# awslabs/dgl-ke

Hardware: NVIDIA H100
Metric: edges/sec TransE_l2 d=400 neg=200 at 1/2/4/8 H100 vs ref CPU; HBM GB/s %peak (higher is better)
Workload: dtype f32

## Files before the change

dgl-ke_b200/csrc/kge_abi.cu:

```cuda
#include <cstdio>
#include <unistd.h>
#include <cstdarg>
#include <cstring>
#include <cstdlib>
#include <map>
#include <mutex>
#include <new>
#include <utility>
#include <cuda.h>
#include "kge_common.cuh"

namespace kge {

namespace {
thread_local char g_err[512] = "";
}

int fail(int code, const char* fmt, ...) {
  va_list ap;
  va_start(ap, fmt);
  vsnprintf(g_err, sizeof(g_err), fmt, ap);
  va_end(ap);
  return code;
}

int smem_optin(const void* kernel, size_t bytes) {
  if (bytes <= 48 * 1024) return KGE_OK;
  if (bytes > kSmemOptinMax) return fail(KGE_ERR_UNSUPPORTED, "%zu bytes of shared memory per CTA requested, sm_90 allows %zu", bytes, kSmemOptinMax);
  int dev = 0;
  cudaGetDevice(&dev);
  static std::mutex mu;
  static std::map<std::pair<const void*, int>, size_t> done;
  std::lock_guard<std::mutex> lock(mu);
  size_t& have = done[{kernel, dev}];
  if (bytes <= have) return KGE_OK;
  const cudaError_t e = cudaFuncSetAttribute(kernel, cudaFuncAttributeMaxDynamicSharedMemorySize, (int)bytes);
  if (e != cudaSuccess) {
    cudaGetLastError();
    return fail(KGE_ERR_CUDA, "cudaFuncSetAttribute(MaxDynamicSharedMemorySize, %zu): %s", bytes, cudaGetErrorString(e));
  }
  have = bytes;
  return KGE_OK;
}

struct Buffer {
  void* p = nullptr;
  size_t bytes = 0;
  bool host = false;
  template <class T> T* as() const { return static_cast<T*>(p); }

  void release() {
    if (p) host ? cudaFreeHost(p) : cudaFree(p);
    p = nullptr;
    bytes = 0;
  }
  int resize(size_t n, cudaStream_t stream, const char* what) {
    cudaStreamCaptureStatus cs = cudaStreamCaptureStatusNone;
    cudaStreamIsCapturing(stream, &cs);
    if (cs != cudaStreamCaptureStatusNone)
      return fail(KGE_ERR_INVALID_ARG, "the %s must be (re)allocated (%zu bytes, has %zu) but the stream is capturing: "
                  "run one eager step first", what, n, bytes);
    cudaError_t e = cudaStreamSynchronize(stream);
    if (e != cudaSuccess) return fail(KGE_ERR_CUDA, "cudaStreamSynchronize before reallocating the %s: %s", what, cudaGetErrorString(e));
    release();
    e = host ? cudaMallocHost(&p, n) : cudaMalloc(&p, n);
    if (e != cudaSuccess) {
      p = nullptr;
      cudaGetLastError();
      return fail(KGE_ERR_NOMEM, "%s(%zu) for the %s failed: %s", host ? "cudaMallocHost" : "cudaMalloc", n, what,
                  cudaGetErrorString(e));
    }
    bytes = n;
    return KGE_OK;
  }
};

}
using namespace kge;

#define KGE_CUDA_OK(expr)                                                                      \
  do {                                                                                         \
    cudaError_t e_ = (expr);                                                                   \
    if (e_ != cudaSuccess) return fail(KGE_ERR_CUDA, "%s: %s", #expr, cudaGetErrorString(e_)); \
  } while (0)

struct kge_context {
  int device = 0;
  int num_sms = 0;
  long long launches = 0;
  int engine = -1;
  int rel_deferred = 0;
  Buffer arena;
  float* ng_ptr = nullptr;
  size_t ng_floats = 0;
  bool ng_dirty = false;
  Buffer pin{nullptr, 0, true};
  Buffer dev_stage;
  float* red_partial = nullptr;
  Buffer rel_dense;
  float* ext_rg = nullptr;
  float* ext_rgs = nullptr;
  float* dump_v = nullptr;
  Buffer negdeg_ids;
  struct Prefetch {
    bool armed = false;
    kge_batch_t next{};
    long long next_nneg = 0;
    bool ready = false;
    const void *r_nodes = nullptr, *r_negs = nullptr, *r_nU_dev = nullptr;
    long long r_nU = 0, r_nneg = 0;
    int r_buf = 0;
    Buffer nc[2];
    Buffer bn[2];
    FusedPrefetch args{};

    void take_staged(const kge_batch_t& b, bool usable, StepParams& p, StepWs& w) {
      if (!ready) return;
      ready = false;
      if (usable && r_nodes == b.node_ids && r_negs == b.neg_ids && r_nU == b.n_nodes &&
          r_nU_dev == (b.n_nodes < 0 ? b.n_nodes_dev : nullptr) && r_nneg == p.Nn) {
        w.NC = nc[r_buf].as<float>();
        w.BnRaw = bn[r_buf].as<float>();
        p.nc_staged = 1;
      }
    }

    int arm_next(bool usable, StepParams& p, StepWs& w, float* arena_nc, cudaStream_t stream, const FusedPrefetch** out) {
      *out = nullptr;
      if (!armed) return KGE_OK;
      armed = false;
      const long long ncap = 2 * p.B;
      const long long nU = next.n_nodes < 0 ? ncap : next.n_nodes;
      if (!usable || nU > ncap || next_nneg <= 0 || fused_prefetch_slots(p, 0) < 2 || fused_prefetch_slots(p, 1) < 2)
        return KGE_OK;
      const size_t ncb = (size_t)ncap * p.D * sizeof(float), bnb = (size_t)next_nneg * p.D * sizeof(float);
      if (ncb > nc[0].bytes || ncb > nc[1].bytes || bnb > bn[0].bytes || bnb > bn[1].bytes) {
        for (int i = 0; i < 2; ++i) {
          int rc;
          if ((rc = nc[i].resize(ncb, stream, "prefetch staging buffers")) || (rc = bn[i].resize(bnb, stream, "prefetch staging buffers")))
            return rc;
        }
        w.BnRaw = nullptr; w.NC = arena_nc; p.nc_staged = 0;
      }
      const int tgt = p.nc_staged ? (r_buf ^ 1) : 0;
      const void* nU_dev = next.n_nodes < 0 ? next.n_nodes_dev : nullptr;
      args = FusedPrefetch{(const long long*)next.node_ids, (const long long*)nU_dev, nU, (const long long*)next.neg_ids,
                           next_nneg, nc[tgt].as<float>(), bn[tgt].as<float>()};
      ready = true;
      r_nodes = next.node_ids; r_negs = next.neg_ids; r_nU = next.n_nodes; r_nU_dev = nU_dev; r_nneg = next_nneg; r_buf = tgt;
      *out = &args;
      return KGE_OK;
    }
  } pf;
  int fused_mode = -1;
  float* dev_log4 = nullptr;
  StepParams last_p{};
  StepWs last_w{};
  BatchView last_b{};
  TableView last_ent{}, last_rel{};
  bool have_last = false;
  Profiler prof;
};

namespace {

struct DeviceGuard {
  int prev = -1;
  explicit DeviceGuard(int dev) {
    cudaGetDevice(&prev);
    if (prev != dev) cudaSetDevice(dev);
    else prev = -1;
  }
  ~DeviceGuard() {
    if (prev >= 0) cudaSetDevice(prev);
  }
};

int make_view(const kge_table_t* t, TableView* v, const char* what) {
  if (!t || !t->shards) return fail(KGE_ERR_INVALID_ARG, "%s table is null", what);
  if (t->n_shards < 1 || t->n_shards > KGE_MAX_SHARDS)
    return fail(KGE_ERR_INVALID_ARG, "%s table: n_shards=%d out of [1,%d]", what, t->n_shards, KGE_MAX_SHARDS);
  if (t->dim <= 0 || t->num_rows <= 0) return fail(KGE_ERR_INVALID_ARG, "%s table: empty", what);
  memset(v, 0, sizeof(*v));
  v->n_shards = t->n_shards;
  v->dim = t->dim;
  v->num_rows = t->num_rows;
  v->rows_per_shard = (t->num_rows + t->n_shards - 1) / t->n_shards;
  for (int s = 0; s < t->n_shards; ++s) {
    const kge_shard_t& sh = t->shards[s];
    long long begin = (long long)s * v->rows_per_shard;
    long long end = begin + v->rows_per_shard;
    if (end > t->num_rows) end = t->num_rows;
    if (sh.row_begin != begin || sh.row_end != end || sh.dim != t->dim)
      return fail(KGE_ERR_INVALID_ARG, "%s table: shard %d must cover rows [%lld,%lld) with dim %d", what, s, begin,
                  end, t->dim);
    if (!sh.emb || !sh.state_sum) return fail(KGE_ERR_INVALID_ARG, "%s table: shard %d has null pointers", what, s);
    if (((uintptr_t)sh.emb & 15) != 0) return fail(KGE_ERR_INVALID_ARG, "%s table: shard %d not 16-byte aligned", what, s);
    v->emb[s] = sh.emb;
    v->state[s] = sh.state_sum;
  }
  return KGE_OK;
}

int make_params(const kge_step_cfg_t* cfg, long long n_nodes, StepParams* p) {
  if (!cfg) return fail(KGE_ERR_INVALID_ARG, "cfg is null");
  if (cfg->model < KGE_TRANSE_L1 || cfg->model > KGE_ROTATE) return fail(KGE_ERR_INVALID_ARG, "unknown model %d", cfg->model);
  if (cfg->batch <= 0 || cfg->chunk_size <= 0 || cfg->neg_sample_size <= 0)
    return fail(KGE_ERR_INVALID_ARG, "batch/chunk_size/neg_sample_size must be positive");
  if (cfg->batch % cfg->chunk_size != 0)
    return fail(KGE_ERR_INVALID_ARG, "batch %lld is not a multiple of chunk_size %d", (long long)cfg->batch, cfg->chunk_size);
  const int D = cfg->entity_dim, Dr = cfg->relation_dim;
  if (D <= 0 || Dr <= 0) return fail(KGE_ERR_INVALID_ARG, "dims must be positive");
  if (D % 4 != 0 || Dr % 4 != 0)
    return fail(KGE_ERR_UNSUPPORTED, "row lengths must be multiples of 4 floats (16-byte vector/TMA access): D_e=%d D_r=%d", D, Dr);
  switch (cfg->model) {
    case KGE_TRANSE_L1: case KGE_TRANSE_L2: case KGE_DISTMULT:
      if (Dr != D) return fail(KGE_ERR_INVALID_ARG, "model needs relation_dim == entity_dim (%d vs %d)", Dr, D);
      break;
    case KGE_COMPLEX:
      if (Dr != D || D % 8 != 0) return fail(KGE_ERR_INVALID_ARG, "ComplEx needs relation_dim == entity_dim, a multiple of 8");
      break;
    case KGE_ROTATE:
      if (D != 2 * Dr || D % 8 != 0) return fail(KGE_ERR_INVALID_ARG, "RotatE needs entity_dim == 2*relation_dim (-de), a multiple of 8");
      break;
    case KGE_RESCAL:
      if (Dr != D * D) return fail(KGE_ERR_INVALID_ARG, "RESCAL needs relation_dim == entity_dim^2");
      if (D > 512) return fail(KGE_ERR_UNSUPPORTED, "RESCAL entity_dim %d > 512 is not implemented", D);
      break;
  }
  p->model = cfg->model; p->D = D; p->Dr = Dr;
  p->gamma = cfg->gamma; p->emb_init = cfg->emb_init; p->lr = cfg->lr;
  p->reg_coef = cfg->reg_coef; p->reg_norm = cfg->reg_norm;
  p->adversarial = cfg->adversarial; p->adv_temperature = cfg->adv_temperature;
  p->neg_head = cfg->neg_head ? 1 : 0;
  p->B = cfg->batch; p->Cs = cfg->chunk_size; p->Ns = cfg->neg_sample_size;
  p->C = (int)(cfg->batch / cfg->chunk_size);
  p->neg_deg = cfg->neg_deg_sample ? 1 : 0;
  if (p->neg_deg) p->Ns += p->Cs;
  p->Nn = (long long)p->C * p->Ns;
  p->U = n_nodes >= 0 ? n_nodes : 2 * p->B;
  p->U_dev = nullptr;
  p->rel_deferred = 0; p->rel_dense = 0; p->use_nc = 1; p->fused = 0; p->nc_staged = 0;
  if (cfg->loss_genre < KGE_LOSS_LOGSIGMOID || cfg->loss_genre > KGE_LOSS_BCE)
    return fail(KGE_ERR_INVALID_ARG, "loss_genre %d is not a kge_loss_t", cfg->loss_genre);
  if (cfg->pairwise && cfg->loss_genre != KGE_LOSS_HINGE && cfg->loss_genre != KGE_LOSS_LOGISTIC)
    return fail(KGE_ERR_INVALID_ARG, "pairwise needs the Hinge or the Logistic criterion (loss.py:61-62)");
  if (cfg->pairwise && cfg->adversarial)
    return fail(KGE_ERR_INVALID_ARG, "loss cannot be pairwise and adversarial sampled (base_loss.py:83-84)");
  p->hinge = cfg->loss_genre == KGE_LOSS_HINGE ? 1 : 0;
  p->margin = cfg->margin;
  p->pairwise = cfg->pairwise ? 1 : 0;
  return KGE_OK;
}

size_t align_up(size_t x, size_t a = 256) { return (x + a - 1) / a * a; }

struct CarveOpt {
  bool force_tiles = false;
  bool want_scores = true;
};

bool use_fused(kge_context* h, const StepParams& p) {
  return h->engine != 0 && h->fused_mode != 0 && fused_supported(p);
}

bool use_umma(kge_context* h, const StepParams& p) {
  return h->engine != 0 && umma_supported(p);
}

int carve(kge_context* h, const StepParams& p, StepWs* w, cudaStream_t stream, const CarveOpt& opt = CarveOpt()) {
  const size_t BD = (size_t)p.B * p.D, ND = (size_t)p.Nn * p.D, BNs = (size_t)p.B * p.Ns;
  const size_t B = (size_t)p.B, Nn = (size_t)p.Nn, U = (size_t)(p.U > 0 ? p.U : 0);
  const bool um = !opt.force_tiles && use_umma(h, p);
  const bool fused = p.fused != 0;
  const size_t sA = B * slab_blocks(p.D) * 32 + 8192, sB = Nn * slab_blocks(p.D) * 32 + 8192;
  const size_t sV = B * slab_blocks(p.Ns) * 32 + 8192;
  const size_t sAT = (size_t)p.C * slab_blocks(p.Cs) * p.D * 32 + 8192, sBT = (size_t)p.C * slab_blocks(p.Ns) * p.D * 32 + 8192;
  const size_t sVT = (size_t)p.C * slab_blocks(p.Cs) * p.Ns * 32 + 8192;
  struct Slot { float** ptr; size_t floats; bool on; };
  const Slot slots[] = {
      {&w->NG, (U ? 2 * B : 0) * p.D, true},
      {&w->A, BD, !(um || fused)}, {&w->Bn, ND, true}, {&w->GA, BD, true}, {&w->GR, B * p.Dr, !p.rel_dense},
      {&w->S, BNs, !fused || opt.want_scores}, {&w->V, BNs, !fused},
      {&w->pos, B, true}, {&w->gpos, B, true}, {&w->pnorm, B, true}, {&w->a2, B, true}, {&w->b2, Nn, true},
      {&w->rowsum, B, true}, {&w->colsum, Nn, true}, {&w->pl, B, true}, {&w->nl, B, true}, {&w->wbar, 4, true},
      {&w->gsr, B, true}, {&w->gsn, Nn, true}, {&w->colpart, (size_t)ceil_div(p.Cs, 128) * Nn, fused},
      {&w->Mt, BD, p.model == KGE_RESCAL},
      {&w->Ahi, sA, um}, {&w->Alo, sA, um}, {&w->Bhi, sB, um}, {&w->Blo, sB, um},
      {&w->Vhi, sV, um && !fused}, {&w->Vlo, sV, um && !fused},
      {&w->AhiT, sAT, um}, {&w->AloT, sAT, um}, {&w->BhiT, sBT, um}, {&w->BloT, sBT, um},
      {&w->VhiT, sVT, um}, {&w->VloT, sVT, um},
      {&w->NC, U * p.D, p.use_nc != 0},
      {&w->regp, B + Nn + (U ? 2 * B : 0), true},
  };
  size_t need = 0;
  for (const Slot& s : slots)
    if (s.on) need += align_up(s.floats * sizeof(float));
  if (need > h->arena.bytes) {
    if (int rc = h->arena.resize(need + need / 4, stream, "step workspace")) return rc;
    h->ng_ptr = nullptr; h->ng_floats = 0;
  }
  size_t off = 0;
  for (const Slot& s : slots) {
    *s.ptr = s.on ? (float*)(h->arena.as<char>() + off) : nullptr;
    if (s.on) off += align_up(s.floats * sizeof(float));
  }
  w->red_partial = h->red_partial; w->red_ticket = (unsigned int*)(h->red_partial + 192);
  w->sync_ctr = (unsigned int*)(h->red_partial + 200);
  w->rg = nullptr; w->rgs = nullptr;
  return KGE_OK;
}

int ensure_rel_dense(kge_context* h, const TableView& rel, StepWs* w, cudaStream_t stream) {
  const size_t bytes = ((size_t)rel.num_rows * rel.dim + (size_t)rel.num_rows) * sizeof(float);
  if (bytes != h->rel_dense.bytes) {
    if (int rc = h->rel_dense.resize(bytes, stream, "relation gradient sums")) return rc;
    KGE_CUDA_OK(cudaMemsetAsync(h->rel_dense.p, 0, bytes, stream));
  }
  w->rg = h->rel_dense.as<float>();
  w->rgs = w->rg + (size_t)rel.num_rows * rel.dim;
  return KGE_OK;
}

LaunchCtx lctx(kge_context* h, void* stream) { return LaunchCtx{(cudaStream_t)stream, &h->launches, h->num_sms, &h->prof}; }

void ensure_ng_zero(kge_context* h, const StepParams& p, const StepWs& w, const LaunchCtx& c, bool force) {
  size_t n = (size_t)2 * p.B * p.D;
  if (force || h->ng_dirty || h->ng_ptr != w.NG || h->ng_floats < n) {
    launch_fill_zero(c, w.NG, (long long)n);
    h->ng_ptr = w.NG;
    h->ng_dirty = false;
  }
  h->ng_floats = n;
}

int check_batch(const kge_batch_t* b, const StepParams& p) {
  if (!b) return fail(KGE_ERR_INVALID_ARG, "batch is null");
  if (!b->node_ids || !b->head_local || !b->tail_local || !b->rel_ids || !b->neg_ids)
    return fail(KGE_ERR_INVALID_ARG, "batch has null index arrays");
  if (b->n_nodes < 0 && b->n_nodes_dev) return KGE_OK;
  if (b->n_nodes <= 0 || b->n_nodes > 2 * p.B) return fail(KGE_ERR_INVALID_ARG, "n_nodes=%lld out of (0, 2*batch]", (long long)b->n_nodes);
  return KGE_OK;
}

BatchView bview(const kge_batch_t* b) {
  return BatchView{(const long long*)b->node_ids, (const long long*)b->head_local, (const long long*)b->tail_local,
                   (const long long*)b->rel_ids, (const long long*)b->neg_ids, b->edge_weight,
                   (const long long*)b->head_ids, (const long long*)b->tail_ids};
}

int run_score(kge_context* h, const LaunchCtx& c, const StepParams& p, const StepWs& w) {
  if (use_umma(h, p)) return umma_score(c, p, w);
  launch_score(c, p, w);
  return KGE_OK;
}

}

extern "C" {

KGE_API int kge_abi_version(void) { return KGE_ABI_VERSION; }
KGE_API const char* kge_last_error(void) { return g_err; }

KGE_API int kge_create(int device, kge_handle_t* out) {
  if (!out) return fail(KGE_ERR_INVALID_ARG, "out is null");
  *out = nullptr;
  int n = 0;
  cudaError_t e = cudaGetDeviceCount(&n);
  if (e != cudaSuccess || n == 0) {
    cudaGetLastError();
    return fail(KGE_ERR_NO_DEVICE, "no CUDA device visible (%s); libkge_b200 has no CPU path", cudaGetErrorString(e));
  }
  if (device < 0 || device >= n) return fail(KGE_ERR_INVALID_ARG, "device %d out of range [0,%d)", device, n);
  cudaDeviceProp prop;
  KGE_CUDA_OK(cudaGetDeviceProperties(&prop, device));
  if (prop.major != 9)
    return fail(KGE_ERR_NO_DEVICE, "device %d is sm_%d%d; this library is built for sm_90a (H100) only", device, prop.major, prop.minor);
  kge_context* h = new (std::nothrow) kge_context();
  if (!h) return fail(KGE_ERR_NOMEM, "out of host memory");
  h->device = device;
  h->num_sms = prop.multiProcessorCount;
  if (const char* ev = getenv("KGE_B200_FUSED")) h->fused_mode = atoi(ev) ? 1 : 0;

  DeviceGuard g(device);
  if (cudaMalloc(&h->dev_log4, 4 * sizeof(float)) != cudaSuccess) { delete h; return fail(KGE_ERR_NOMEM, "cudaMalloc failed"); }

  if (cudaMalloc(&h->red_partial, 256 * sizeof(float)) != cudaSuccess || cudaMemset(h->red_partial, 0, 256 * sizeof(float)) != cudaSuccess) {
    delete h; return fail(KGE_ERR_NOMEM, "cudaMalloc failed");
  }
  *out = h;
  return KGE_OK;
}

KGE_API int kge_destroy(kge_handle_t h) {
  if (!h) return KGE_OK;
  DeviceGuard g(h->device);
  cudaDeviceSynchronize();
  for (Buffer* b : {&h->arena, &h->dev_stage, &h->pin, &h->rel_dense, &h->negdeg_ids, &h->pf.nc[0], &h->pf.nc[1],
                    &h->pf.bn[0], &h->pf.bn[1]})
    b->release();
  if (h->dev_log4) cudaFree(h->dev_log4);
  if (h->red_partial) cudaFree(h->red_partial);
  if (h->prof.created)
    for (int i = 0; i < Profiler::kMax; ++i) { cudaEventDestroy(h->prof.ev0[i]); cudaEventDestroy(h->prof.ev1[i]); }
  delete h;
  return KGE_OK;
}

KGE_API int64_t kge_launch_count(kge_handle_t h) { return h ? h->launches : 0; }

KGE_API int kge_profile_enable(kge_handle_t h, int on) {
  if (!h) return fail(KGE_ERR_INVALID_ARG, "handle is null");
  DeviceGuard g(h->device);
  Profiler& p = h->prof;
  if (on && !p.created) {
    for (int i = 0; i < Profiler::kMax; ++i) {
      KGE_CUDA_OK(cudaEventCreate(&p.ev0[i]));
      KGE_CUDA_OK(cudaEventCreate(&p.ev1[i]));
    }
    p.created = true;
  }
  p.enabled = on != 0;
  p.n = 0;
  return KGE_OK;
}

KGE_API int kge_profile_read(kge_handle_t h, char* names, int names_len, float* ms, int max_records) {
  if (!h || !names || !ms) return fail(KGE_ERR_INVALID_ARG, "null argument");
  DeviceGuard g(h->device);
  Profiler& p = h->prof;
  KGE_CUDA_OK(cudaDeviceSynchronize());
  int n = p.n < max_records ? p.n : max_records, off = 0;
  names[0] = 0;
  for (int i = 0; i < n; ++i) {
    KGE_CUDA_OK(cudaEventElapsedTime(&ms[i], p.ev0[i], p.ev1[i]));
    int w = snprintf(names + off, names_len - off, "%s%s", i ? "|" : "", p.names[i]);
    if (w < 0 || off + w >= names_len) break;
    off += w;
  }
  p.n = 0;
  return n;
}

KGE_API int kge_set_engine(kge_handle_t h, int engine) {
  if (!h) return fail(KGE_ERR_INVALID_ARG, "handle is null");
  if (engine < -1 || engine > 1) return fail(KGE_ERR_INVALID_ARG, "engine must be -1, 0 or 1");
  h->engine = engine;
  return KGE_OK;
}

KGE_API int kge_set_fused(kge_handle_t h, int mode) {
  if (!h) return fail(KGE_ERR_INVALID_ARG, "handle is null");
  if (mode < -1 || mode > 1) return fail(KGE_ERR_INVALID_ARG, "mode must be -1, 0 or 1");
  h->fused_mode = mode;
  return KGE_OK;
}

KGE_API int kge_debug_set_dump(kge_handle_t h, float* coef_dump) {
  if (!h) return fail(KGE_ERR_INVALID_ARG, "handle is null");
  h->dump_v = coef_dump;
  return KGE_OK;
}

KGE_API int kge_gather(kge_handle_t h, const kge_table_t* table, const int64_t* idx, int64_t n, float* out, void* stream) {
  if (!h) return fail(KGE_ERR_INVALID_ARG, "handle is null");
  if (n < 0) return fail(KGE_ERR_INVALID_ARG, "n < 0");
  if (n == 0) return KGE_OK;
  if (!idx || !out) return fail(KGE_ERR_INVALID_ARG, "idx/out is null");
  TableView v;
  int rc = make_view(table, &v, "gather");
  if (rc) return rc;
  DeviceGuard g(h->device);
  launch_gather(lctx(h, stream), v, (const long long*)idx, n, out);
  KGE_CUDA_OK(cudaGetLastError());
  return KGE_OK;
}

KGE_API int kge_score_pos(kge_handle_t h, const kge_step_cfg_t* cfg, const float* head, const float* rel, const float* tail,
                  int64_t n, float* out, void* stream) {
  if (!h) return fail(KGE_ERR_INVALID_ARG, "handle is null");
  if (!cfg) return fail(KGE_ERR_INVALID_ARG, "cfg is null");
  if (n == 0) return KGE_OK;
  if (!head || !rel || !tail || !out || n < 0) return fail(KGE_ERR_INVALID_ARG, "bad arguments");
  kge_step_cfg_t c2 = *cfg;
  c2.batch = n; c2.chunk_size = (int32_t)1; c2.neg_sample_size = 1;
  if (n > 0x7fffffffLL) return fail(KGE_ERR_INVALID_ARG, "n too large");
  StepParams p;
  int rc = make_params(&c2, 0, &p);
  if (rc) return rc;
  DeviceGuard g(h->device);
  StepWs w{};
  w.pos = out;
  LaunchCtx c = lctx(h, stream);
  if (p.model == KGE_RESCAL) launch_rescal_prep_dense(c, p, head, rel, tail, w, true, false);
  else launch_prep_dense(c, p, head, rel, tail, nullptr, w, true, false);
  KGE_CUDA_OK(cudaGetLastError());
  return KGE_OK;
}

KGE_API int kge_score_neg(kge_handle_t h, const kge_step_cfg_t* cfg, const float* heads, const float* rel, const float* tails,
                  float* out, void* stream) {
  if (!h) return fail(KGE_ERR_INVALID_ARG, "handle is null");
  if (!heads || !rel || !tails || !out) return fail(KGE_ERR_INVALID_ARG, "null pointer");
  StepParams p;
  int rc = make_params(cfg, 0, &p);
  if (rc) return rc;
  DeviceGuard g(h->device);
  StepWs w{};
  CarveOpt opt;
  opt.force_tiles = (p.model == KGE_RESCAL);
  rc = carve(h, p, &w, (cudaStream_t)stream, opt);
  if (rc) return rc;
  h->ng_ptr = nullptr;
  LaunchCtx c = lctx(h, stream);
  const float* negrows = p.neg_head ? heads : tails;
  if (p.model == KGE_RESCAL) launch_rescal_prep_dense(c, p, heads, rel, tails, w, false, true);
  else launch_prep_dense(c, p, heads, rel, tails, negrows, w, false, true);
  StepWs w2 = w;
  w2.Bn = const_cast<float*>(negrows);
  w2.S = out;
  if (opt.force_tiles) launch_score(c, p, w2);
  else rc = run_score(h, c, p, w2);
  if (rc) return rc;
  KGE_CUDA_OK(cudaGetLastError());
  h->have_last = false;
  return KGE_OK;
}

KGE_API int kge_loss_grad(kge_handle_t h, const kge_step_cfg_t* cfg, const float* pos, const float* neg, const float* wt,
                  float* dpos, float* dneg, float* log4, void* stream) {
  if (!h) return fail(KGE_ERR_INVALID_ARG, "handle is null");
  if (!pos || !neg || !dpos || !dneg) return fail(KGE_ERR_INVALID_ARG, "null pointer");
  StepParams p;
  int rc = make_params(cfg, 0, &p);
  if (rc) return rc;
  p.model = KGE_DISTMULT;
  DeviceGuard g(h->device);
  StepWs w{};
  rc = carve(h, p, &w, (cudaStream_t)stream);
  if (rc) return rc;
  h->ng_ptr = nullptr;
  w.V = dneg;
  w.gpos = dpos;
  launch_loss(lctx(h, stream), p, pos, neg, wt, w, log4, false);
  KGE_CUDA_OK(cudaGetLastError());
  h->have_last = false;
  return KGE_OK;
}

KGE_API int kge_adagrad(kge_handle_t h, const kge_table_t* table, const int64_t* idx, const float* grad, int64_t n, float lr,
                void* stream) {
  if (!h) return fail(KGE_ERR_INVALID_ARG, "handle is null");
  if (n < 0) return fail(KGE_ERR_INVALID_ARG, "n < 0");
  if (n == 0) return KGE_OK;
  if (!idx || !grad) return fail(KGE_ERR_INVALID_ARG, "null pointer");
  TableView v;
  int rc = make_view(table, &v, "adagrad");
  if (rc) return rc;
  DeviceGuard g(h->device);
  launch_adagrad(lctx(h, stream), v, (const long long*)idx, grad, n, lr);
  KGE_CUDA_OK(cudaGetLastError());
  return KGE_OK;
}

static int forward_backward_impl(kge_handle_t h, const kge_step_cfg_t* cfg, const kge_table_t* ent, const kge_table_t* rel,
                                 const kge_batch_t* batch, float* log4, void* stream, bool fused_step) {
  if (!h) return fail(KGE_ERR_INVALID_ARG, "handle is null");
  StepParams p;
  int rc = make_params(cfg, batch ? batch->n_nodes : 0, &p);
  if (rc) return rc;
  rc = check_batch(batch, p);
  if (rc) return rc;
  if (batch->n_nodes < 0) p.U_dev = (const long long*)batch->n_nodes_dev;
  p.rel_deferred = h->rel_deferred;
  TableView ve, vr;
  if ((rc = make_view(ent, &ve, "entity"))) return rc;
  if ((rc = make_view(rel, &vr, "relation"))) return rc;
  if (ve.dim != p.D || vr.dim != p.Dr)
    return fail(KGE_ERR_INVALID_ARG, "table dims (%d,%d) do not match cfg (%d,%d)", ve.dim, vr.dim, p.D, p.Dr);
  DeviceGuard g(h->device);
  p.fused = use_fused(h, p) ? 1 : 0;
  p.use_nc = (fused_step && ve.n_shards == 1) ? 0 : 1;
  p.rel_dense = (fused_step && p.model != KGE_RESCAL &&
                 (p.rel_deferred ? (h->ext_rg != nullptr) : ((size_t)vr.num_rows * (size_t)vr.dim <= ((size_t)64 << 20)))) ? 1 : 0;
  StepWs w{};
  CarveOpt opt;
  opt.want_scores = !fused_step;
  if ((rc = carve(h, p, &w, (cudaStream_t)stream, opt))) return rc;
  if (p.rel_dense && p.rel_deferred) { w.rg = h->ext_rg; w.rgs = h->ext_rgs; }
  else if (p.rel_dense && (rc = ensure_rel_dense(h, vr, &w, (cudaStream_t)stream))) return rc;
  LaunchCtx c = lctx(h, stream);
  BatchView b = bview(batch);
  if (p.neg_deg) {
    if (ve.n_shards != 1) return fail(KGE_ERR_UNSUPPORTED, "--neg_deg_sample needs a single-shard entity table");
// ... 478 lines not shown
```

dgl-ke_b200/csrc/kge_common.cuh:

```cuda
#pragma once
#include <cuda_runtime.h>
#include <stdint.h>
#include "../../include/kge_b200.h"

namespace kge {

constexpr int kWarp = 32;

struct TableView {
  float* emb[KGE_MAX_SHARDS];
  float* state[KGE_MAX_SHARDS];
  long long rows_per_shard;
  long long num_rows;
  int n_shards;
  int dim;
};

__device__ __forceinline__ float* row_ptr(const TableView& t, long long id) {
  if (t.n_shards == 1) return t.emb[0] + id * (long long)t.dim;
  int s = (int)(id / t.rows_per_shard);
  return t.emb[s] + (id - (long long)s * t.rows_per_shard) * (long long)t.dim;
}
__device__ __forceinline__ float* state_ptr(const TableView& t, long long id) {
  if (t.n_shards == 1) return t.state[0] + id;
  int s = (int)(id / t.rows_per_shard);
  return t.state[s] + (id - (long long)s * t.rows_per_shard);
}

struct StepParams {
  int model;
  int D;
  int Dr;
  float gamma, emb_init, lr, reg_coef;
  int reg_norm;
  int adversarial;
  float adv_temperature;
  int neg_head;
  long long B;
  int C, Cs, Ns;
  long long Nn;
  long long U;
  const long long* U_dev;
  int rel_deferred;
  int rel_dense;
  int use_nc;
  int fused;
  int hinge;
  float margin;
  int pairwise;
  int neg_deg;
  int nc_staged;
};

__host__ __device__ __forceinline__ bool node_reg_in_update(const StepParams& p) { return !p.use_nc || p.nc_staged; }

struct StepWs {
  float* A;
  float* Bn;
  float* GA;
  float* GR;
  float* NG;
  float* NC;
  float* S;
  float* V;
  float* pos;
  float* gpos;
  float* pnorm;
  float* a2;
  float* b2;
  float* rowsum;
  float* colsum;
  float* pl;
  float* nl;
  float* regp;
  float* wbar;
  float* gsr;
  float* gsn;
  float* colpart;
  float* rg;
  float* rgs;
  const float* BnRaw;
  unsigned int* sync_ctr;
  float* red_partial;
  unsigned int* red_ticket;
  float* Mt;
  float *Ahi, *Alo;
  float *Bhi, *Blo;
  float *Vhi, *Vlo;
  float *AhiT, *AloT;
  float *BhiT, *BloT;
  float *VhiT, *VloT;
};

struct BatchView {
  const long long* node_ids;
  const long long* head_local;
  const long long* tail_local;
  const long long* rel_ids;
  const long long* neg_ids;
  const float* edge_weight;
  const long long* head_ids;
  const long long* tail_ids;
};

__device__ __forceinline__ long long node_count(const StepParams& p) { return p.U_dev ? *p.U_dev : p.U; }

__device__ __forceinline__ const float* node_row(const StepParams& p, const TableView& ent, const BatchView& b,
                                                 const StepWs& w, long long loc) {
  return p.use_nc ? (w.NC + loc * (long long)p.D) : row_ptr(ent, b.node_ids[loc]);
}
__device__ __forceinline__ const float* head_row(const StepParams& p, const TableView& ent, const BatchView& b,
                                                 const StepWs& w, long long i) {
  if (!p.use_nc && b.head_ids) return row_ptr(ent, b.head_ids[i]);
  return node_row(p, ent, b, w, b.head_local[i]);
}
__device__ __forceinline__ const float* tail_row(const StepParams& p, const TableView& ent, const BatchView& b,
                                                 const StepWs& w, long long i) {
  if (!p.use_nc && b.tail_ids) return row_ptr(ent, b.tail_ids[i]);
  return node_row(p, ent, b, w, b.tail_local[i]);
}

__device__ __forceinline__ float warp_sum(float v) {
#pragma unroll
  for (int o = 16; o > 0; o >>= 1) v += __shfl_xor_sync(0xffffffffu, v, o);
  return v;
}
__device__ __forceinline__ float warp_max(float v) {
#pragma unroll
  for (int o = 16; o > 0; o >>= 1) v = fmaxf(v, __shfl_xor_sync(0xffffffffu, v, o));
  return v;
}

__device__ __forceinline__ float4 ld4(const float* p) { return *reinterpret_cast<const float4*>(p); }
__device__ __forceinline__ void st4(float* p, float4 v) { *reinterpret_cast<float4*>(p) = v; }
__device__ __forceinline__ float4 ld4_stream(const float* p) {
  float4 r;
  asm volatile("ld.global.L1::no_allocate.v4.f32 {%0,%1,%2,%3}, [%4];"
               : "=f"(r.x), "=f"(r.y), "=f"(r.z), "=f"(r.w) : "l"(p));
  return r;
}
__device__ __forceinline__ void red_add4(float* p, float4 v) {
  asm volatile("red.global.add.v4.f32 [%0], {%1,%2,%3,%4};"
               :: "l"(p), "f"(v.x), "f"(v.y), "f"(v.z), "f"(v.w) : "memory");
}

__device__ __forceinline__ void red_add4_sys(float* p, float4 v) {
  asm volatile("red.relaxed.sys.global.add.v4.f32 [%0], {%1,%2,%3,%4};"
               :: "l"(p), "f"(v.x), "f"(v.y), "f"(v.z), "f"(v.w) : "memory");
}
__device__ __forceinline__ void table_red_add4(const TableView& t, float* p, float4 v) {
  if (t.n_shards > 1) red_add4_sys(p, v); else red_add4(p, v);
}
__device__ __forceinline__ void table_atomic_add(const TableView& t, float* p, float v) {
  if (t.n_shards > 1) atomicAdd_system(p, v); else atomicAdd(p, v);
}

#define KGE_F4_OP2(name, expr)                                                     \
  __device__ __forceinline__ float4 name(float4 a, float4 b) {                     \
    float4 r;                                                                      \
    { float x = a.x, y = b.x; r.x = (expr); } { float x = a.y, y = b.y; r.y = (expr); } \
    { float x = a.z, y = b.z; r.z = (expr); } { float x = a.w, y = b.w; r.w = (expr); } \
    return r;                                                                      \
  }
KGE_F4_OP2(f4_add, x + y)
KGE_F4_OP2(f4_sub, x - y)
KGE_F4_OP2(f4_mul, x* y)
#undef KGE_F4_OP2
__device__ __forceinline__ float4 f4_scale(float4 a, float s) { return make_float4(a.x * s, a.y * s, a.z * s, a.w * s); }
__device__ __forceinline__ float4 f4_neg(float4 a) { return make_float4(-a.x, -a.y, -a.z, -a.w); }
__device__ __forceinline__ float4 f4_fma(float4 a, float s, float4 c) {
  return make_float4(fmaf(a.x, s, c.x), fmaf(a.y, s, c.y), fmaf(a.z, s, c.z), fmaf(a.w, s, c.w));
}
__device__ __forceinline__ float f4_hsum(float4 a) { return (a.x + a.y) + (a.z + a.w); }
__device__ __forceinline__ float f4_dot(float4 a, float4 b) { return f4_hsum(f4_mul(a, b)); }
__device__ __forceinline__ float sgnf(float x) { return (x > 0.f) ? 1.f : ((x < 0.f) ? -1.f : 0.f); }

__device__ __forceinline__ void split_tf32(float x, float& hi, float& lo) {
  uint32_t hb, lb;
  asm("cvt.rna.tf32.f32 %0, %1;" : "=r"(hb) : "f"(x));
  hi = __uint_as_float(hb);
  asm("cvt.rna.tf32.f32 %0, %1;" : "=r"(lb) : "f"(x - hi));
  lo = __uint_as_float(lb);
}
__device__ __forceinline__ void split_tf32_4(float4 v, float4& h, float4& l) {
  split_tf32(v.x, h.x, l.x); split_tf32(v.y, h.y, l.y); split_tf32(v.z, h.z, l.z); split_tf32(v.w, h.w, l.w);
}
__host__ __device__ inline int slab_blocks(int ncol) { return (ncol + 31) >> 5; }
__device__ __forceinline__ long long slab_off(long long chunk, int nblk, int R, int row, int col) {
  return ((chunk * nblk + (col >> 5)) * (long long)R + row) * 32 + (col & 31);
}
__device__ __forceinline__ long long slabT_off(long long chunk, int R, int Ncol, int row, int col) {
  return ((chunk * slab_blocks(R) + (row >> 5)) * (long long)Ncol + col) * 32 + (row & 31);
}
constexpr int kPrepRows = 32;
constexpr size_t kSmemOptinMax = 227 * 1024;
__host__ __device__ inline int prep_stage_stride(int D) { return ((D + 27) & ~31) + 4; }
inline size_t prep_stage_bytes(int D) { return (size_t)kPrepRows * prep_stage_stride(D) * sizeof(float); }
inline bool prep_stage_fits(int D) { return prep_stage_bytes(D) <= kSmemOptinMax; }

struct RowOut {
  float* f32;
  float* hi;
  float* lo;
  long long chunk;
  int nblk, R, row;
  float* stage;
};
__device__ __forceinline__ void row_store4(const RowOut& o, int col, float4 v) {
  if (o.f32) *reinterpret_cast<float4*>(o.f32 + col) = v;
  if (o.hi) {
    float4 h, l;
    split_tf32_4(v, h, l);
    const long long off = slab_off(o.chunk, o.nblk, o.R, o.row, col);
    *reinterpret_cast<float4*>(o.hi + off) = h;
    *reinterpret_cast<float4*>(o.lo + off) = l;
  }
  if (o.stage) *reinterpret_cast<float4*>(o.stage + col) = v;
}

static __device__ __noinline__ float abs_pow_generic(float ax, int p) { return powf(ax, (float)p); }
__device__ __forceinline__ float abs_pow(float x, int p) {
  float ax = fabsf(x);
  if (p == 3) return ax * ax * ax;
  if (p == 2) return ax * ax;
  if (p == 1) return ax;
  return abs_pow_generic(ax, p);
}
static __device__ __noinline__ float reg_grad_pow(float x, int p, float coef) {
  return coef * (float)p * powf(fabsf(x), (float)(p - 1)) * sgnf(x);
}
__device__ __forceinline__ float reg_grad(float x, int p, float coef) {
  if (coef == 0.f || p <= 0) return 0.f;
  float ax = fabsf(x);
  if (p == 3) return 3.f * coef * ax * x;
  if (p == 2) return 2.f * coef * x;
  if (p == 1) return coef * sgnf(x);
  return reg_grad_pow(x, p, coef);
}
__device__ __forceinline__ float4 reg_grad4(float4 x, int p, float coef) {
  return make_float4(reg_grad(x.x, p, coef), reg_grad(x.y, p, coef), reg_grad(x.z, p, coef), reg_grad(x.w, p, coef));
}
__device__ __forceinline__ float abs_pow4_sum(float4 x, int p) {
  return (abs_pow(x.x, p) + abs_pow(x.y, p)) + (abs_pow(x.z, p) + abs_pow(x.w, p));
}

__device__ __forceinline__ float softplusf(float s) { return fmaxf(s, 0.f) + log1pf(expf(-fabsf(s))); }
__device__ __forceinline__ float sigmoidf(float s) {
  if (s >= 0.f) return 1.f / (1.f + expf(-s));
  float e = expf(s);
  return e / (1.f + e);
}

inline int ceil_div(long long a, long long b) { return (int)((a + b - 1) / b); }

int fail(int code, const char* fmt, ...);
int smem_optin(const void* kernel, size_t bytes);

struct Profiler {
  static constexpr int kMax = 64;
  bool enabled = false;
  int n = 0;
  const char* names[kMax];
  cudaEvent_t ev0[kMax], ev1[kMax];
  bool created = false;
};

struct LaunchCtx {
  cudaStream_t stream;
  long long* launch_counter;
  int num_sms;
  Profiler* prof;
};

inline void prof_begin(const LaunchCtx& c, const char* name) {
  Profiler* p = c.prof;
  if (!p || !p->enabled || p->n >= Profiler::kMax) return;
  p->names[p->n] = name;
  cudaEventRecord(p->ev0[p->n], c.stream);
}
inline void prof_end(const LaunchCtx& c) {
  Profiler* p = c.prof;
  if (!p || !p->enabled || p->n >= Profiler::kMax) return;
  cudaEventRecord(p->ev1[p->n], c.stream);
  ++p->n;
}

#define KGE_LAUNCH_NAMED(ctx, name, kernel, grid, block, smem, ...)            \
  do {                                                                          \
    prof_begin((ctx), name);                                                    \
    kernel<<<(grid), (block), (smem), (ctx).stream>>>(__VA_ARGS__);             \
    prof_end((ctx));                                                            \
    if ((ctx).launch_counter) ++*(ctx).launch_counter;                          \
  } while (0)

#define KGE_LAUNCH(ctx, kernel, grid, block, smem, ...)                         \
  do {                                                                          \
    prof_begin((ctx), #kernel);                                                 \
    kernel<<<(grid), (block), (smem), (ctx).stream>>>(__VA_ARGS__);             \
    prof_end((ctx));                                                            \
    if ((ctx).launch_counter) ++*(ctx).launch_counter;                          \
  } while (0)

struct SamplerParams {
  const long long *heads, *rels, *tails;
  long long n_edges, n_entities;
  long long B, Nn;
  unsigned long long seed;
  int half_bits;
  long long *o_head, *o_rel, *o_tail;
  long long *o_neg;
  long long *o_nodes, *o_hl, *o_tl;
  long long* o_n_nodes;
  unsigned long long* tkey;
  int* tpos;
  int* tloc;
  int hmask;
  int* flags;
};

void launch_sampler(const LaunchCtx&, const SamplerParams&, long long step);

void launch_gather(const LaunchCtx&, const TableView& t, const long long* idx, long long n, float* out);
void launch_gather_nodes(const LaunchCtx&, const StepParams&, const TableView& ent, const BatchView&, const StepWs&);
int launch_prep(const LaunchCtx&, const StepParams&, const TableView& ent, const TableView& rel,
                const BatchView&, const StepWs&);
int launch_prep_nonedge(const LaunchCtx&, const StepParams&, const TableView& ent, const TableView& rel,
                        const BatchView&, const StepWs&);
void launch_prep_dense(const LaunchCtx&, const StepParams&, const float* head, const float* relr,
                       const float* tail, const float* negrows, const StepWs&, bool want_pos, bool want_a);
void launch_score(const LaunchCtx&, const StepParams&, const StepWs&);
void launch_loss(const LaunchCtx&, const StepParams&, const float* pos, const float* S, const float* w,
                 const StepWs&, float* log4, bool want_reg);
void launch_wbar(const LaunchCtx&, const StepParams&, const float* w, const StepWs&);
void launch_loss_rows(const LaunchCtx&, const StepParams&, const float* pos, const float* S, const float* w, const StepWs&);
void launch_colsum(const LaunchCtx&, const StepParams&, const StepWs&);
void launch_reduce_log(const LaunchCtx&, const StepParams&, const float* w, const StepWs&, float* log4, bool want_reg);
void launch_grad_a(const LaunchCtx&, const StepParams&, const StepWs&);
void launch_grad_b(const LaunchCtx&, const StepParams&, const StepWs&);
void launch_chain(const LaunchCtx&, const StepParams&, const TableView& ent, const TableView& rel,
                  const BatchView&, const StepWs&);
int launch_update(const LaunchCtx&, const StepParams&, const TableView& ent, const TableView& rel,
                  const BatchView&, const StepWs&, float* log4, const float* wt);
void launch_adagrad(const LaunchCtx&, const TableView& t, const long long* idx, const float* grad,
                    long long n, float lr);
void launch_node_grad_with_reg(const LaunchCtx&, const StepParams&, const TableView& ent,
                               const BatchView&, const StepWs&, float* out);
void launch_fill_zero(const LaunchCtx&, float* p, long long n);
void launch_rel_grad_dense(const LaunchCtx&, const StepParams&, const BatchView&, const StepWs&, float* rg, float* rgs);
void launch_rel_apply_dense(const LaunchCtx&, const TableView& rel, float* rg, float* rgs, float lr);

void launch_negdeg_ids(const LaunchCtx&, const StepParams&, const BatchView&, const long long* sampled, long long* out);
void launch_negdeg_zero_reg(const LaunchCtx&, const StepParams&, const StepWs&);
void launch_negdeg_mask_scores(const LaunchCtx&, const StepParams&, const StepWs&);
void launch_negdeg_mask_coef(const LaunchCtx&, const StepParams&, const StepWs&);
void launch_negdeg_scatter(const LaunchCtx&, const StepParams&, const TableView& ent, const BatchView&, const StepWs&);

int launch_rescal_prep(const LaunchCtx&, const StepParams&, const TableView& ent, const TableView& rel,
                       const BatchView&, const StepWs&);
void launch_rescal_prep_dense(const LaunchCtx&, const StepParams&, const float* head, const float* relr,
                              const float* tail, const StepWs&, bool want_pos, bool want_a);
void launch_rescal_chain(const LaunchCtx&, const StepParams&, const TableView& ent, const TableView& rel,
                         const BatchView&, const StepWs&);

bool umma_supported(const StepParams&);
int umma_score(const LaunchCtx&, const StepParams&, const StepWs&);
int umma_grad(const LaunchCtx&, const StepParams&, const StepWs&, bool side_b);

struct FusedPrefetch {
  const long long* node_ids;
  const long long* nU_dev;
  long long nU;
  const long long* neg_ids;
  long long nNeg;
  float* nc;
  float* bn;
};
bool fused_supported(const StepParams&);
int fused_prefetch_slots(const StepParams& p, int mode);
int fused_launch(const LaunchCtx&, const StepParams&, const StepWs&, int mode, const float* wt, float* dumpS, float* dumpV,
                 const TableView* ent, const long long* neg_ids, const FusedPrefetch* pf);

}
```

dgl-ke_b200/csrc/kge_fused.cu:

```cuda
#include <cuda.h>
#include <cstdio>
#include <cstdlib>
#include <mutex>
#include "kge_common.cuh"
#include "kge_tc.cuh"

namespace kge {

using namespace tc;

namespace {

constexpr int kTileM = 128;
constexpr int kThreadsF = 384;
constexpr int kProducerWarp = 8;
constexpr int kHandoffWarp = 9;
constexpr int kMaxS1 = 4, kMaxS2 = 8;
constexpr int kMaxPf = 8;
constexpr uint32_t kRingBytes = 192 * 1024;
constexpr uint32_t kRingBytesP = 223 * 1024;
constexpr float kLog2e = 1.4426950408889634f;
constexpr float kLn2 = 0.6931471805599453f;

struct FusedArgs {
  int model, adversarial;
  float gamma, Tl2e, inv2B, uni;
  float reg_coef;
  int reg_norm;
  int C, Rx, Ry, D;
  int N1;
  int N2;
  int nblkD;
  int nS1, nS2;
  uint32_t stage1Bytes, stage2Bytes;
  float *VhiT, *VloT;
  float* colpart;
  int ncolpart;
  const float* x2;
  const float* y2;
  const float* pos;
  const float* wt;
  const float* wbar;
  float *gpos, *rowsum, *pl, *nl;
  float* dumpS;
  float* dumpV;
  const float *Xhi, *Xlo;
  const long long* xids;
  TableView xtab;
  const float* xraw;
  float* gsn;
  float* out;
  int pf_slots;
  int pf_parity;
  int pf_lag;
  uint32_t pf_off, pf_row_bytes;
  const long long* pf_node_ids;
  const long long* pf_nU_dev;
  long long pf_nU, pf_nNeg;
  const long long* pf_neg_ids;
  float* pf_nc;
  float* pf_bn;
};

static __device__ __noinline__ float reg_grad_any(float b, int norm, float coef) { return reg_grad(b, norm, coef); }
__device__ __forceinline__ float reg_grad_fast(float b, int norm, float coef) {
  if (norm == 3) return 3.f * coef * fabsf(b) * b;
  return reg_grad_any(b, norm, coef);
}

__device__ __forceinline__ void epi_bar() { asm volatile("bar.sync 1, 256;" ::: "memory"); }

__device__ __forceinline__ void prefetch_rows(const FusedArgs& g, uint8_t* ring, uint64_t (*pf_full)[kMaxPf], int w, int lane) {
  const int S = g.pf_slots;
  const long long nU = g.pf_nU_dev ? *g.pf_nU_dev : g.pf_nU;
  const long long total = nU + g.pf_nNeg;
  const long long nhalf = total > g.pf_parity ? (total - g.pf_parity + 1) / 2 : 0;
  const long long stride = 2ll * gridDim.x, j0 = 2ll * blockIdx.x + w;
  const long long n = j0 < nhalf ? (nhalf - j0 + stride - 1) / stride : 0;
  uint8_t* slots = ring + g.pf_off + (size_t)w * S * g.pf_row_bytes;
  auto vrow = [&](long long k) { return g.pf_parity + 2 * (j0 + k * stride); };
  auto fetch_ids = [&](long long kb) {
    const long long k = kb + lane;
    if (k >= n) return 0ll;
    const long long v = vrow(k);
    return v < nU ? g.pf_node_ids[v] : g.pf_neg_ids[v - nU];
  };
  long long ids_lo = fetch_ids(0), ids_hi = fetch_ids(32);
  long long base = 0;
  auto load = [&](long long k) {
    const int o = (int)(k - base);
    const long long id = __shfl_sync(0xffffffffu, o < 32 ? ids_lo : ids_hi, o & 31);
    const int s = (int)(k % S);
    if (elect_one()) {
      mbar_expect_tx(&pf_full[w][s], g.pf_row_bytes);
      bulk_g2s(slots + (size_t)s * g.pf_row_bytes, row_ptr(g.xtab, id), g.pf_row_bytes, &pf_full[w][s]);
    }
    __syncwarp();
  };
  for (long long k = 0; k < n && k < S; ++k) load(k);
  const int L = g.pf_lag < S - 1 ? g.pf_lag : (S > 2 ? S - 2 : 1);
  for (long long k = 0; k < n; ++k) {
    const int s = (int)(k % S);
    mbar_wait(&pf_full[w][s], (uint32_t)((k / S) & 1));
    const long long v = vrow(k);
    float* dst = v < nU ? g.pf_nc + v * (long long)g.D : g.pf_bn + (v - nU) * (long long)g.D;
    const long long kr = k - L + S;
    const bool reload = k >= L && kr < n;
    if (reload && kr >= base + 32) { base += 32; ids_lo = ids_hi; ids_hi = fetch_ids(base + 32); }
    if (elect_one()) {
      bulk_s2g(dst, slots + (size_t)s * g.pf_row_bytes, g.pf_row_bytes);
      bulk_commit();
      if (reload) { if (L == 3) bulk_wait_read<3>(); else if (L == 2) bulk_wait_read<2>(); else bulk_wait_read<1>(); }
    }
    __syncwarp();
    if (reload) load(kr);
  }
  if (elect_one()) bulk_wait_all();
  __syncwarp();
}

template <int NW, int KS>
__device__ __forceinline__ void kblock_3xtf32(float (&acc)[NW / 2], uint64_t dXh, uint64_t dXl, uint64_t dYh, uint64_t dYl) {
  wgmma_fence();
#pragma unroll
  for (int ks = 0; ks < KS; ++ks) {
    const uint64_t o = (uint64_t)(ks * 2);
    wgmma_ss<NW>(acc, dXh + o, dYh + o, 1u);
    wgmma_ss<NW>(acc, dXh + o, dYl + o, 1u);
    wgmma_ss<NW>(acc, dXl + o, dYh + o, 1u);
  }
  wgmma_commit();
}

template <int NV>
__device__ __forceinline__ int vsm_idx(int i, int k) {
  const int g = i & 7, h = (i >> 3) & 1, kk = k & 7;
  const int L = 4 * g + (kk & 3);
  return (((i >> 4) * (NV / 8) + (k >> 3)) * 32 + (L ^ ((L >> 3) & 3))) * 4 + h + 2 * (kk >> 2);
}

template <int NW>
__device__ __forceinline__ void pos_kstep(float (&acc2)[NW / 2], uint32_t (&ah)[4], uint32_t (&al)[4], const float* vf,
                                          uint64_t dYh, uint64_t dYl) {
  const float4 v = *reinterpret_cast<const float4*>(vf);
  const float a[4] = {v.x, v.y, v.z, v.w};
#pragma unroll
  for (int r = 0; r < 4; ++r) {
    float hi, lo;
    split_tf32(a[r], hi, lo);
    ah[r] = __float_as_uint(hi); al[r] = __float_as_uint(lo);
  }
  wgmma_fence();
  wgmma_rs<NW>(acc2, ah, dYh, 1u);
  wgmma_rs<NW>(acc2, ah, dYl, 1u);
  wgmma_rs<NW>(acc2, al, dYh, 1u);
  wgmma_commit();
}

__device__ __forceinline__ int tile_row() {
  uint32_t t;
  asm volatile("mov.u32 %0, %%tid.x;" : "=r"(t));
  return (int)((t >> 5) * 16 + ((t >> 2) & 7));
}

template <int NV, int NW>
__global__ void __launch_bounds__(kThreadsF, 1)
k_fused_pos(const __grid_constant__ CUtensorMap mXh, const __grid_constant__ CUtensorMap mXl,
            const __grid_constant__ CUtensorMap mYh1, const __grid_constant__ CUtensorMap mYl1,
            const __grid_constant__ CUtensorMap mYh2, const __grid_constant__ CUtensorMap mYl2, FusedArgs g) {
  extern __shared__ __align__(1024) uint8_t smem_raw[];
  __shared__ __align__(8) uint64_t full1[kMaxS1], empty1[kMaxS1], full2[kMaxS2], empty2[kMaxS2];
  __shared__ __align__(8) uint64_t vfree;
  __shared__ __align__(8) uint64_t pf_full[2][kMaxPf];
  __shared__ __align__(16) float colA[NV];
  __shared__ float rsc[kTileM];

  const int warp = threadIdx.x >> 5, lane = threadIdx.x & 31;
  uint8_t* ring = (uint8_t*)(((uintptr_t)smem_raw + 1023) & ~(uintptr_t)1023);
  float* vsm = reinterpret_cast<float*>(ring);
  constexpr uint32_t vBytes = (uint32_t)NV * 512u;
  uint8_t* ring2 = ring + vBytes;

  const int mtiles = (g.Rx + kTileM - 1) / kTileM;
  const int ntiles = g.C * mtiles;
  const int nkb1 = (g.D + 31) >> 5;
  const int nkb2 = (g.Ry + 31) >> 5;
  const int nchunks = (g.D + NW - 1) / NW;
  constexpr uint32_t yBytes1 = (uint32_t)NV * 128u;
  constexpr uint32_t yBytes2 = (uint32_t)NW * 128u;
  const bool l2 = g.model == KGE_TRANSE_L2;
  const int nhand = g.pf_slots > 0 ? 1 : 3;
  const uint32_t hand_bar_n = 256u + 32u * (uint32_t)nhand;

  if (threadIdx.x == 0) {
    for (int s = 0; s < kMaxS1; ++s) { mbar_init(&full1[s], 1); mbar_init(&empty1[s], 8); }
    for (int s = 0; s < kMaxS2; ++s) { mbar_init(&full2[s], 1); mbar_init(&empty2[s], 8); }
    mbar_init(&vfree, 8 + nhand);
    for (int s = 0; s < kMaxPf; ++s) { mbar_init(&pf_full[0][s], 1); mbar_init(&pf_full[1][s], 1); }
    asm volatile("fence.mbarrier_init.release.cluster;" ::: "memory");
  }
  if (warp == kProducerWarp && lane == 0) {
    tma_prefetch_desc(&mXh); tma_prefetch_desc(&mXl); tma_prefetch_desc(&mYh1);
    tma_prefetch_desc(&mYl1); tma_prefetch_desc(&mYh2); tma_prefetch_desc(&mYl2);
  }
  __syncthreads();

  if (warp >= 8) {
  asm volatile("setmaxnreg.dec.sync.aligned.u32 56;");
  if (warp == kProducerWarp) {
    uint32_t n1 = 0, n2 = 0, it = 0;
    for (int tile = blockIdx.x; tile < ntiles; tile += gridDim.x, ++it) {
      const int c = tile / mtiles, m0 = (tile % mtiles) * kTileM;
      if (it > 0) mbar_wait(&vfree, (it - 1) & 1);
      for (int kb = 0; kb < nkb1; ++kb, ++n1) {
        const uint32_t s = n1 % g.nS1;
        mbar_wait(&empty1[s], ((n1 / g.nS1) & 1) ^ 1);
        uint8_t* st = ring + (size_t)s * g.stage1Bytes;
        const int yx = (c * g.nblkD + kb) * g.Rx + m0;
        const int yy = (c * g.nblkD + kb) * g.Ry;
        if (elect_one()) {
          mbar_expect_tx(&full1[s], 2u * 16384u + 2u * yBytes1);
          tma_load_2d(st, &mXh, &full1[s], 0, yx);
          tma_load_2d(st + 16384, &mXl, &full1[s], 0, yx);
          tma_load_2d(st + 32768, &mYh1, &full1[s], 0, yy);
          tma_load_2d(st + 32768 + yBytes1, &mYl1, &full1[s], 0, yy);
        }
        __syncwarp();
      }
      for (uint32_t k = (n1 > (uint32_t)g.nS1 ? n1 - g.nS1 : 0); k < n1; ++k) mbar_wait(&empty1[k % g.nS1], (k / g.nS1) & 1);
      for (int ch = 0; ch < nchunks; ++ch) {
        for (int kb = 0; kb < nkb2; ++kb, ++n2) {
          const uint32_t s = n2 % g.nS2;
          mbar_wait(&empty2[s], ((n2 / g.nS2) & 1) ^ 1);
          uint8_t* st = ring2 + (size_t)s * g.stage2Bytes;
          const int yy = (c * nkb2 + kb) * g.D + ch * NW;
          if (elect_one()) {
            mbar_expect_tx(&full2[s], 2u * yBytes2);
            tma_load_2d(st, &mYh2, &full2[s], 0, yy);
            tma_load_2d(st + yBytes2, &mYl2, &full2[s], 0, yy);
          }
          __syncwarp();
        }
      }
    }
  } else if (warp - kHandoffWarp < nhand) {
    const int hw = warp - kHandoffWarp;
    for (int tile = blockIdx.x; tile < ntiles; tile += gridDim.x) {
      const int c = tile / mtiles, m0 = (tile % mtiles) * kTileM;
      const int rows = g.Rx - m0 < kTileM ? g.Rx - m0 : kTileM;
      const int nb = (rows + 31) >> 5;
      asm volatile("bar.sync 2, %0;" ::"r"(hand_bar_n) : "memory");
      float* dst = g.colpart + (long long)(tile % mtiles) * g.C * g.Ry + (long long)c * g.Ry;
      for (int j = hw; j < g.Ry; j += nhand) {
        float s = 0.f;
        float v[kTileM / 32];
#pragma unroll
        for (int b = 0; b < kTileM / 32; ++b) {
          const int i = 32 * b + lane;
          v[b] = b < nb ? vsm[vsm_idx<NV>(i, j)] * rsc[i] : 0.f;
        }
#pragma unroll
        for (int b = 0; b < kTileM / 32; ++b) {
          const int i = 32 * b + lane;
          if (i < rows) {
            float hi, lo;
            split_tf32(v[b], hi, lo);
            const long long o = slabT_off(c, g.Rx, g.Ry, m0 + i, j);
            g.VhiT[o] = hi; g.VloT[o] = lo;
          }
          s += v[b];
        }
        if (l2) {
#pragma unroll
          for (int x = 16; x >= 1; x >>= 1) s += __shfl_xor_sync(0xffffffffu, s, x);
          if (lane == 0) dst[j] = s;
        }
      }
      asm volatile("fence.proxy.async.shared::cta;" ::: "memory");
      __syncwarp();
      if (lane == 0) mbar_arrive(&vfree);
    }
  } else if (warp >= 10 && g.pf_slots > 0) {
    prefetch_rows(g, ring, pf_full, warp - 10, lane);
  }
  } else {
    asm volatile("setmaxnreg.inc.sync.aligned.u32 224;");
    const int wg = warp >> 2, q = lane & 3;
    const int et = threadIdx.x;
    uint32_t n1 = 0, n2 = 0;
    for (int tile = blockIdx.x; tile < ntiles; tile += gridDim.x) {
      const int c = tile / mtiles, m0 = (tile % mtiles) * kTileM;
      epi_bar();
      for (int y = et; y < NV; y += 256) {
        const bool ok = y < g.Ry;
        colA[y] = (l2 && ok) ? g.y2[(long long)c * g.Ry + y] : 0.f;
      }
      epi_bar();
      float rscal[2];
      {
      float acc[NV / 2];
#pragma unroll
      for (int i = 0; i < NV / 2; ++i) acc[i] = 0.f;
      for (int kb = 0; kb < nkb1; ++kb, ++n1) {
        const uint32_t s = n1 % g.nS1;
        mbar_wait(&full1[s], (n1 / g.nS1) & 1);
        const uint32_t st = smem_u32(ring + (size_t)s * g.stage1Bytes);
        const uint64_t dXh = make_desc(st + wg * 8192u), dXl = make_desc(st + 16384u + wg * 8192u);
        const uint64_t dYh = make_desc(st + 32768u), dYl = make_desc(st + 32768u + yBytes1);
        const int kleft = g.D - kb * 32;
        const int ksteps = kleft >= 32 ? 4 : (kleft >> 3);
        switch (ksteps) {
          case 4: kblock_3xtf32<NV, 4>(acc, dXh, dXl, dYh, dYl); break;
          case 3: kblock_3xtf32<NV, 3>(acc, dXh, dXl, dYh, dYl); break;
          case 2: kblock_3xtf32<NV, 2>(acc, dXh, dXl, dYh, dYl); break;
          default: kblock_3xtf32<NV, 1>(acc, dXh, dXl, dYh, dYl); break;
        }
        if (kb > 0) {
          wgmma_wait<1>();
          if (lane == 0) mbar_arrive(&empty1[(n1 - 1) % g.nS1]);
        }
      }
      wgmma_wait<0>();
      if (lane == 0) mbar_arrive(&empty1[(n1 - 1) % g.nS1]);
      reg_fence(acc);
      epi_bar();
      const int rloc = tile_row();

#pragma unroll
      for (int h = 0; h < 2; ++h) {
        const int m = m0 + rloc + 8 * h;
        const bool row_ok = m < g.Rx;
        const long long gx = (long long)c * g.Rx + (row_ok ? m : 0);
        const float x2v = (l2 && row_ok) ? g.x2[gx] : 0.f;
        const float w_i = (g.wt && row_ok) ? g.wt[gx] : 1.f;
        const float kw = w_i * g.inv2B;
        float mxl = -INFINITY;
        if (g.adversarial || g.dumpS) {
#pragma unroll
          for (int j = 0; j < NV / 8; ++j) {
            float sv[2];
#pragma unroll
            for (int e = 0; e < 2; ++e) {
              const int col = 8 * j + 2 * q + e;
              float s = acc[4 * j + 2 * h + e];
              if (l2) {
                const float sqc = fmaxf(fmaf(-2.f, s, colA[col]) + x2v, 1e-30f);
                s = g.gamma - sqc * rsqrta(sqc);
              }
              sv[e] = s;
              if (col < g.Ry) mxl = fmaxf(mxl, s * g.Tl2e);
            }
            if (g.dumpS && row_ok && 8 * j + 2 * q < g.Ry)
              *reinterpret_cast<float2*>(g.dumpS + gx * g.Ry + 8 * j + 2 * q) = make_float2(sv[0], sv[1]);
          }
        }
        if (g.adversarial) {
          mxl = fmaxf(mxl, __shfl_xor_sync(0xffffffffu, mxl, 1));
          mxl = fmaxf(mxl, __shfl_xor_sync(0xffffffffu, mxl, 2));
        } else {
          mxl = 0.f;
        }
        float nls = 0.f, rs = 0.f, den = 0.f;
#pragma unroll
        for (int j = 0; j < NV / 8; ++j) {
#pragma unroll
          for (int e = 0; e < 2; ++e) {
            const int col = 8 * j + 2 * q + e;
            float s = acc[4 * j + 2 * h + e], rinv = 1.f;
            if (l2) {
              const float sq = fmaf(-2.f, s, colA[col]) + x2v;
              const float sqc = fmaxf(sq, 1e-30f);
              const float r = rsqrta(sqc);
              s = g.gamma - sqc * r;
              rinv = (sq > 1e-30f) ? r : 0.f;
            }
            const float pe = g.adversarial ? ex2a(fmaf(s, g.Tl2e, -mxl)) : 1.f;
            const float t = ex2a(-fabsf(s) * kLog2e);
            const float u = 1.f + t;
            const float r1 = rcpa(u);
            const float sig = (s >= 0.f) ? r1 : t * r1;
            const float sp = fmaf(kLn2, lg2a(u), fmaxf(s, 0.f));
            const bool ok = row_ok && (col < g.Ry);
            const float coef = ok ? pe * sig * kw * rinv : 0.f;
            if (ok) { nls = fmaf(pe, sp, nls); den += pe; }
            rs += coef;
            vsm[vsm_idx<NV>(rloc + 8 * h, col)] = coef;
          }
        }
        den += __shfl_xor_sync(0xffffffffu, den, 1); den += __shfl_xor_sync(0xffffffffu, den, 2);
        nls += __shfl_xor_sync(0xffffffffu, nls, 1); nls += __shfl_xor_sync(0xffffffffu, nls, 2);
        rs += __shfl_xor_sync(0xffffffffu, rs, 1); rs += __shfl_xor_sync(0xffffffffu, rs, 2);
        const float rscale = g.adversarial ? (row_ok ? 1.f / den : 0.f) : g.uni;
        rscal[h] = rscale;
        if (g.dumpV && row_ok) {
          for (int j = 0; j < NV / 8; ++j)
            if (8 * j + 2 * q < g.Ry)
              *reinterpret_cast<float2*>(g.dumpV + gx * g.Ry + 8 * j + 2 * q) =
                  make_float2(vsm[vsm_idx<NV>(rloc + 8 * h, 8 * j + 2 * q)] * rscale,
                              vsm[vsm_idx<NV>(rloc + 8 * h, 8 * j + 2 * q + 1)] * rscale);
        }
        if (q == 0 && row_ok) {
          const float ps = g.pos[gx];
          const float wb = g.wt ? *g.wbar : 1.f;
          g.pl[gx] = softplusf(-ps);
          g.nl[gx] = nls * rscale * w_i;
          g.gpos[gx] = -sigmoidf(-ps) * wb * g.inv2B;
          if (l2) g.rowsum[gx] = rs * rscale;
        }
      }
      if (q == 0) { rsc[rloc] = rscal[0]; rsc[rloc + 8] = rscal[1]; }
      }
      asm volatile("bar.arrive 2, %0;" ::"r"(hand_bar_n) : "memory");
      __syncwarp();

      const float* vw = vsm + ((warp * (NV / 8)) * 32 + (lane ^ ((lane >> 3) & 3))) * 4;
      const int rloc = tile_row();
      for (int ch = 0; ch < nchunks; ++ch) {
        const int d0 = ch * NW;
        float acc2[NW / 2];
#pragma unroll
        for (int i = 0; i < NW / 2; ++i) acc2[i] = 0.f;
        uint32_t ah[2][4], al[2][4];
#pragma unroll 1
        for (int kb = 0; kb < nkb2; ++kb) {
          const uint32_t s = n2 % g.nS2;
          mbar_wait(&full2[s], (n2 / g.nS2) & 1);
          const uint32_t st = smem_u32(ring2 + (size_t)s * g.stage2Bytes);
          const uint64_t dYh = make_desc(st), dYl = make_desc(st + yBytes2);
          const int kleft = g.Ry - kb * 32;
          const int ksteps = kleft >= 32 ? 4 : (kleft >> 3);
#pragma unroll
          for (int ks = 0; ks < 4; ++ks) {
            const int j = kb * 4 + ks;
            if (ks < ksteps) {
              const uint64_t o = (uint64_t)(ks * 2);
              pos_kstep<NW>(acc2, ah[j & 1], al[j & 1], vw + j * 128, dYh + o, dYl + o);
              if (j > 0) {
                wgmma_wait<1>();
                reg_fence(ah[(j - 1) & 1]); reg_fence(al[(j - 1) & 1]);
                if (ks == 0 && lane == 0) mbar_arrive(&empty2[(n2 - 1) % g.nS2]);
              }
            }
          }
          ++n2;
        }
        wgmma_wait<0>();
        reg_fence(ah[0]); reg_fence(ah[1]); reg_fence(al[0]); reg_fence(al[1]);
        if (lane == 0) mbar_arrive(&empty2[(n2 - 1) % g.nS2]);
        reg_fence(acc2);
#pragma unroll
        for (int h = 0; h < 2; ++h) {
          const int m = m0 + rloc + 8 * h;
          if (m >= g.Rx) continue;
          float* orow = g.out + ((long long)c * g.Rx + m) * (long long)g.D;
#pragma unroll
          for (int j = 0; j < NW / 8; ++j) {
            const int k = d0 + 8 * j + 2 * q;
            if (k >= g.D) continue;
            *reinterpret_cast<float2*>(orow + k) = make_float2(acc2[4 * j + 2 * h] * rscal[h], acc2[4 * j + 2 * h + 1] * rscal[h]);
          }
        }
      }
      asm volatile("fence.proxy.async.shared::cta;" ::: "memory");
      __syncwarp();
      if (lane == 0) mbar_arrive(&vfree);
    }
  }
}

constexpr int kNegEpiLoads = 16;

template <int NW, bool FLAT>
__global__ void __launch_bounds__(kThreadsF, 1)
k_fused_neg(const __grid_constant__ CUtensorMap mVh, const __grid_constant__ CUtensorMap mVl,
            const __grid_constant__ CUtensorMap mAh, const __grid_constant__ CUtensorMap mAl, FusedArgs g) {
  extern __shared__ __align__(1024) uint8_t smem_raw[];
  __shared__ __align__(8) uint64_t full[kMaxS1], empty[kMaxS1];
  __shared__ __align__(8) uint64_t pf_full[2][kMaxPf];

  const int warp = threadIdx.x >> 5, lane = threadIdx.x & 31;
  uint8_t* ring = (uint8_t*)(((uintptr_t)smem_raw + 1023) & ~(uintptr_t)1023);

  const int mtiles = (g.Rx + kTileM - 1) / kTileM;
  const int ntiles = g.C * mtiles;
  const int nkb = (g.Ry + 31) >> 5;
  const int nch = (g.D + NW - 1) / NW;
  constexpr uint32_t aBytes = (uint32_t)kTileM * 128u;
  constexpr uint32_t bBytes = (uint32_t)NW * 128u;
  const bool l2 = g.model == KGE_TRANSE_L2;

  if (threadIdx.x == 0) {
    for (int s = 0; s < kMaxS1; ++s) { mbar_init(&full[s], 1); mbar_init(&empty[s], 8); }
    for (int s = 0; s < kMaxPf; ++s) { mbar_init(&pf_full[0][s], 1); mbar_init(&pf_full[1][s], 1); }
    asm volatile("fence.mbarrier_init.release.cluster;" ::: "memory");
  }
  if (warp == kProducerWarp && lane == 0) {
    tma_prefetch_desc(&mVh); tma_prefetch_desc(&mVl); tma_prefetch_desc(&mAh); tma_prefetch_desc(&mAl);
  }
  __syncthreads();

  if (warp >= 8) {
  asm volatile("setmaxnreg.dec.sync.aligned.u32 56;");
  if (warp == kProducerWarp) {
    uint32_t n = 0;
    for (int tile = blockIdx.x; tile < ntiles; tile += gridDim.x) {
      const int c = tile / mtiles, m0 = (tile % mtiles) * kTileM;
      for (int ch = 0; ch < nch; ++ch) {
        for (int kb = 0; kb < nkb; ++kb, ++n) {
          const uint32_t s = n % g.nS1;
          mbar_wait(&empty[s], ((n / g.nS1) & 1) ^ 1);
          uint8_t* st = ring + (size_t)s * g.stage1Bytes;
          const int yv = (c * nkb + kb) * g.Rx + m0;
          const int ya = (c * nkb + kb) * g.D + ch * NW;
          if (elect_one()) {
            mbar_expect_tx(&full[s], 2u * aBytes + 2u * bBytes);
            tma_load_2d(st, &mVh, &full[s], 0, yv);
            tma_load_2d(st + aBytes, &mVl, &full[s], 0, yv);
            tma_load_2d(st + 2 * aBytes, &mAh, &full[s], 0, ya);
            tma_load_2d(st + 2 * aBytes + bBytes, &mAl, &full[s], 0, ya);
          }
          __syncwarp();
        }
      }
    }
  } else if (warp >= 10 && g.pf_slots > 0) {
    prefetch_rows(g, ring, pf_full, warp - 10, lane);
  }
  } else {
    asm volatile("setmaxnreg.inc.sync.aligned.u32 224;");
    const int wg = warp >> 2, q = lane & 3;
    const int et = threadIdx.x;
    const int rloc = wg * 64 + (warp & 3) * 16 + (lane >> 2);
    uint32_t n = 0;
    for (int tile = blockIdx.x; tile < ntiles; tile += gridDim.x) {
      const int c = tile / mtiles, m0 = (tile % mtiles) * kTileM;
      if (g.dumpV) {
        for (int e = et; e < kTileM * g.Ry; e += 256) {
          const int j = m0 + e / g.Ry, i = e % g.Ry;
          if (j >= g.Rx) break;
          const long long o = slabT_off(c, g.Ry, g.Rx, i, j);
          g.dumpV[((long long)c * g.Rx + j) * g.Ry + i] = g.VhiT[o] + g.VloT[o];
        }
      }
      float cs[2] = {0.f, 0.f};
      if (l2) {
#pragma unroll
        for (int h = 0; h < 2; ++h) {
          const int m = m0 + rloc + 8 * h;
          if (m >= g.Rx) continue;
          const float* p = g.colpart + (long long)c * g.Rx + m;
          for (int t = 0; t < g.ncolpart; ++t) cs[h] += p[(long long)t * g.C * g.Rx];
        }
      }
      bool rok[2];
      const float* brow[2] = {nullptr, nullptr};
      long long boff[2] = {0, 0};
#pragma unroll
      for (int h = 0; h < 2; ++h) {
        const int m = m0 + rloc + 8 * h;
        rok[h] = m < g.Rx;
        if (!rok[h]) continue;
        const long long gx = (long long)c * g.Rx + m;
        if (FLAT) brow[h] = g.xraw ? g.xraw + gx * (long long)g.D : row_ptr(g.xtab, g.xids[gx]);
        else boff[h] = slab_off(c, g.nblkD, g.Rx, m, 0);
      }
      const long long blk = 32ll * g.Rx;
      constexpr int NJ = NW / 8;
      constexpr int NB = FLAT ? kNegEpiLoads : kNegEpiLoads / 2;
      constexpr bool early = FLAT || NW < 256;
      float2 bh[NB], bl[NB];
      auto load_b = [&](int h, int d0, int j0) {
#pragma unroll
        for (int jj = 0; jj < NB; ++jj) {
          const int k = d0 + 8 * (j0 + jj) + 2 * q;
          if (j0 + jj >= NJ || k >= g.D || !rok[h]) continue;
          if (FLAT) {
            bh[jj] = __ldg(reinterpret_cast<const float2*>(brow[h] + k));
          } else {
            const long long so = boff[h] + (k >> 5) * blk + (k & 31);
            bh[jj] = __ldg(reinterpret_cast<const float2*>(g.Xhi + so));
            bl[jj] = __ldg(reinterpret_cast<const float2*>(g.Xlo + so));
          }
        }
      };
      float gsq[2] = {0.f, 0.f};
      for (int ch = 0; ch < nch; ++ch) {
        const int d0 = ch * NW;
        float acc[NW / 2];
#pragma unroll
        for (int i = 0; i < NW / 2; ++i) acc[i] = 0.f;
        for (int kb = 0; kb < nkb; ++kb, ++n) {
          const uint32_t s = n % g.nS1;
          mbar_wait(&full[s], (n / g.nS1) & 1);
          const uint32_t st = smem_u32(ring + (size_t)s * g.stage1Bytes);
          const uint64_t dVh = make_desc(st + wg * 8192u), dVl = make_desc(st + aBytes + wg * 8192u);
          const uint64_t dAh = make_desc(st + 2 * aBytes), dAl = make_desc(st + 2 * aBytes + bBytes);
          const int kleft = g.Ry - kb * 32;
          const int ksteps = kleft >= 32 ? 4 : (kleft >> 3);
          switch (ksteps) {
            case 4: kblock_3xtf32<NW, 4>(acc, dVh, dVl, dAh, dAl); break;
            case 3: kblock_3xtf32<NW, 3>(acc, dVh, dVl, dAh, dAl); break;
            case 2: kblock_3xtf32<NW, 2>(acc, dVh, dVl, dAh, dAl); break;
            default: kblock_3xtf32<NW, 1>(acc, dVh, dVl, dAh, dAl); break;
          }
          if (kb > 0) {
            wgmma_wait<1>();
            if (lane == 0) mbar_arrive(&empty[(n - 1) % g.nS1]);
          }
        }
        if (early) load_b(0, d0, 0);
        wgmma_wait<0>();
        if (lane == 0) mbar_arrive(&empty[(n - 1) % g.nS1]);
        reg_fence(acc);
#pragma unroll
        for (int h = 0; h < 2; ++h) {
          if (!rok[h]) continue;
          float* orow = g.out + ((long long)c * g.Rx + m0 + rloc + 8 * h) * (long long)g.D;
#pragma unroll
          for (int j0 = 0; j0 < NJ; j0 += NB) {
            if (!early || h > 0 || j0 > 0) load_b(h, d0, j0);
#pragma unroll
            for (int jj = 0; jj < NB; ++jj) {
              const int j = j0 + jj;
              const int k = d0 + 8 * j + 2 * q;
              if (j >= NJ || k >= g.D) continue;
              float o0 = acc[4 * j + 2 * h], o1 = acc[4 * j + 2 * h + 1];
              const float2 b = FLAT ? bh[jj] : make_float2(bh[jj].x + bl[jj].x, bh[jj].y + bl[jj].y);
              if (l2) { o0 = fmaf(b.x, -cs[h], o0); o1 = fmaf(b.y, -cs[h], o1); }
              o0 += reg_grad_fast(b.x, g.reg_norm, g.reg_coef);
              o1 += reg_grad_fast(b.y, g.reg_norm, g.reg_coef);
              gsq[h] += o0 * o0 + o1 * o1;
              *reinterpret_cast<float2*>(orow + k) = make_float2(o0, o1);
            }
          }
        }
      }
#pragma unroll
      for (int h = 0; h < 2; ++h) {
        float v = gsq[h];
        v += __shfl_xor_sync(0xffffffffu, v, 1);
        v += __shfl_xor_sync(0xffffffffu, v, 2);
        const int m = m0 + rloc + 8 * h;
        if (q == 0 && m < g.Rx) g.gsn[(long long)c * g.Rx + m] = v / (float)g.D;
      }
    }
  }
}

}

bool fused_supported(const StepParams& p) {
  return umma_supported(p) && !p.hinge && !p.pairwise && !p.neg_deg && p.Cs <= 240 && p.Ns <= 240;
}

namespace {
struct Geometry { int Rx, Ry, N1, N2, nS1, nS2, pf_slots; uint32_t ringBytes, stage1Bytes, stage2Bytes, pf_off; bool ok; };

int neg_chunk_width(int D, bool want_prefetch) {
  static const int widths[] = {64, 128, 200, 256};
  int best = 0;
  long long best_rows = 0;
  for (int w : widths) {
    if (w == 256 && want_prefetch) continue;
    const long long rows = (long long)((D + w - 1) / w) * (kTileM + w);
    if (!best || rows < best_rows) { best = w; best_rows = rows; }
  }
  return best;
}

Geometry geometry(const StepParams& p, int mode, bool want_prefetch) {
  Geometry q{};
  const uint32_t row = (uint32_t)p.D * 4u;
  if (mode == 1) {
    q.Rx = p.Ns; q.Ry = p.Cs;
    q.ringBytes = kRingBytes;
    q.N1 = neg_chunk_width(p.D, want_prefetch);
    q.stage1Bytes = 2u * kTileM * 128u + 2u * (uint32_t)q.N1 * 128u;
    q.nS1 = (int)(kRingBytes / q.stage1Bytes); if (q.nS1 > kMaxS1) q.nS1 = kMaxS1;
    q.ok = q.nS1 >= 2;
    if (q.ok && want_prefetch) {
      int nS = q.nS1;
      while (nS > 2 && kRingBytes - (uint32_t)nS * q.stage1Bytes < 2u * kMaxPf * row) --nS;
      const uint32_t used = (uint32_t)nS * q.stage1Bytes;
      int slots = (int)((kRingBytes - used) / (2u * row));
      if (slots > kMaxPf) slots = kMaxPf;
      if (slots >= 2) { q.pf_slots = slots; q.nS1 = nS; q.pf_off = used; }
    }
    return q;
  }
  q.Rx = p.Cs; q.Ry = p.Ns;
  q.N1 = q.Ry <= 64 ? 64 : (q.Ry <= 128 ? 128 : (q.Ry <= 208 ? 208 : 256));
  const uint32_t ring = want_prefetch ? kRingBytes : kRingBytesP;
  q.ringBytes = ring;
  q.stage1Bytes = 2u * 16384u + 2u * (uint32_t)q.N1 * 128u;
  int nS1 = (int)(ring / q.stage1Bytes); if (nS1 > kMaxS1) nS1 = kMaxS1;
  if (nS1 < 2) return q;
  const uint32_t vBytes = (uint32_t)q.N1 * 512u;
  const bool w200 = (p.D + 199) / 200 * 200 < (p.D + 127) / 128 * 128;
  const int widths[2] = {w200 ? 200 : 128, w200 ? 128 : 200};
  Geometry first{};
  for (int NW : widths) {
    Geometry t = q;
    t.N2 = NW;
    t.stage2Bytes = 2u * (uint32_t)NW * 128u;
    if (vBytes + 2u * t.stage2Bytes > ring) continue;
    t.nS1 = nS1;
    t.nS2 = (int)((ring - vBytes) / t.stage2Bytes); if (t.nS2 > kMaxS2) t.nS2 = kMaxS2;
    t.ok = true;
    if (!want_prefetch) return t;
    if (!first.ok) first = t;
    const uint32_t want = 2u * kMaxPf * row;
    int s1 = t.nS1, s2 = t.nS2;
    while (s1 > 2 && ring - (uint32_t)s1 * q.stage1Bytes < want) --s1;
    while (s2 > 2 && ring - (vBytes + (uint32_t)s2 * t.stage2Bytes) < want) --s2;
    uint32_t used = (uint32_t)s1 * q.stage1Bytes;
    if (vBytes + (uint32_t)s2 * t.stage2Bytes > used) used = vBytes + (uint32_t)s2 * t.stage2Bytes;
    int slots = (int)((ring - used) / (2u * row));
    if (slots > kMaxPf) slots = kMaxPf;
    if (slots >= 2) { t.pf_slots = slots; t.nS1 = s1; t.nS2 = s2; t.pf_off = used; return t; }
  }
  return first;
}

int launch_error() {
  const cudaError_t e = cudaGetLastError();
  return e == cudaSuccess ? KGE_OK : fail(KGE_ERR_CUDA, "k_fused launch: %s", cudaGetErrorString(e));
}
const char* pos_launch_name(int NV, int NW, int pf) {
  static const int nvs[4] = {64, 128, 208, 256}, nws[2] = {128, 200};
  static char names[4][2][kMaxPf + 1][96];
  static std::once_flag once;
  std::call_once(once, [] {
    for (int a = 0; a < 4; ++a)
      for (int b = 0; b < 2; ++b)
        for (int f = 0; f <= kMaxPf; ++f)
          snprintf(names[a][b][f], sizeof(names[a][b][f]), "k_fused<P: S=A.Bn^T, loss, GA=V.Bn> NV=%d NW=%d pf=%d hand=%d",
                   nvs[a], nws[b], f, f > 0 ? 1 : 3);
  });
  const int a = NV == 64 ? 0 : NV == 128 ? 1 : NV == 208 ? 2 : 3;
  return names[a][NW == 200][pf < 0 ? 0 : (pf > kMaxPf ? kMaxPf : pf)];
}
template <int NV, int NW>
int launch_pos(const LaunchCtx& c, int grid, size_t smem, const CUtensorMap* m, const FusedArgs& g) {
  if (int rc = smem_optin((const void*)k_fused_pos<NV, NW>, smem)) return rc;
  KGE_LAUNCH_NAMED(c, pos_launch_name(NV, NW, g.pf_slots), (k_fused_pos<NV, NW>), grid, kThreadsF, smem,
                   m[0], m[1], m[2], m[3], m[4], m[5], g);
  return launch_error();
}
template <int NV>
int launch_pos(const LaunchCtx& c, int grid, size_t smem, const CUtensorMap* m, const FusedArgs& g) {
  if constexpr (NV < 256) {
    if (g.N2 == 200) return launch_pos<NV, 200>(c, grid, smem, m, g);
  }
  return launch_pos<NV, 128>(c, grid, smem, m, g);
}
template <int NW, bool FLAT>
int launch_neg_src(const LaunchCtx& c, int grid, size_t smem, const CUtensorMap* m, const FusedArgs& g) {
  if (int rc = smem_optin((const void*)k_fused_neg<NW, FLAT>, smem)) return rc;
  KGE_LAUNCH_NAMED(c, "k_fused<N: G_neg=V^T.A, mean sq>", (k_fused_neg<NW, FLAT>), grid, kThreadsF, smem, m[0], m[1], m[2], m[3], g);
  return launch_error();
}
template <int NW>
int launch_neg(const LaunchCtx& c, int grid, size_t smem, const CUtensorMap* m, const FusedArgs& g) {
  return (g.xraw || g.xids) ? launch_neg_src<NW, true>(c, grid, smem, m, g) : launch_neg_src<NW, false>(c, grid, smem, m, g);
}
int launch_width(const LaunchCtx& c, bool P, int grid, size_t smem, const CUtensorMap* m, const FusedArgs& g) {
  switch (g.N1) {
    case 64: return P ? launch_pos<64>(c, grid, smem, m, g) : launch_neg<64>(c, grid, smem, m, g);
    case 128: return P ? launch_pos<128>(c, grid, smem, m, g) : launch_neg<128>(c, grid, smem, m, g);
    case 200: return launch_neg<200>(c, grid, smem, m, g);
    case 208: return launch_pos<208>(c, grid, smem, m, g);
    default: return P ? launch_pos<256>(c, grid, smem, m, g) : launch_neg<256>(c, grid, smem, m, g);
  }
}
}

int fused_prefetch_slots(const StepParams& p, int mode) { return geometry(p, mode, true).pf_slots; }

int fused_launch(const LaunchCtx& c, const StepParams& p, const StepWs& w, int mode, const float* wt, float* dumpS,
                 float* dumpV, const TableView* ent, const long long* neg_ids, const FusedPrefetch* pf) {
  FusedArgs g{};
  g.model = p.model; g.adversarial = p.adversarial;
  g.gamma = p.gamma; g.Tl2e = p.adv_temperature * kLog2e; g.inv2B = 0.5f / (float)p.B; g.uni = 1.f / (float)p.Ns;
  g.reg_coef = p.reg_coef; g.reg_norm = p.reg_norm;
  g.C = p.C; g.D = p.D; g.nblkD = slab_blocks(p.D);
  const bool P = mode == 0;
  const Geometry q = geometry(p, mode, pf != nullptr && ent != nullptr);
  if (!q.ok) return fail(KGE_ERR_UNSUPPORTED, "fused kernel: shape does not fit (N1=%d)", q.N1);
  g.Rx = q.Rx; g.Ry = q.Ry; g.N1 = q.N1; g.N2 = q.N2; g.nS1 = q.nS1; g.nS2 = q.nS2;
  g.stage1Bytes = q.stage1Bytes; g.stage2Bytes = q.stage2Bytes;
  if (pf && ent && q.pf_slots >= 2) {
    static const int lag_env = getenv("KGE_B200_PF_LAG") ? atoi(getenv("KGE_B200_PF_LAG")) : 1;
    g.pf_lag = lag_env < 1 ? 1 : (lag_env > 3 ? 3 : lag_env);
    g.pf_slots = q.pf_slots; g.pf_off = q.pf_off; g.pf_row_bytes = (uint32_t)p.D * 4u; g.pf_parity = mode;
    g.pf_node_ids = pf->node_ids; g.pf_nU_dev = pf->nU_dev; g.pf_nU = pf->nU; g.pf_nNeg = pf->nNeg;
    g.pf_neg_ids = pf->neg_ids; g.pf_nc = pf->nc; g.pf_bn = pf->bn;
    g.xtab = *ent;
  }
  g.VhiT = w.VhiT; g.VloT = w.VloT; g.colpart = w.colpart; g.ncolpart = (p.Cs + kTileM - 1) / kTileM;
  g.dumpV = dumpV;
  const size_t smem = q.ringBytes + 1024;
  const int mtiles = (g.Rx + kTileM - 1) / kTileM;
  int grid = p.C * mtiles;
  if (grid > c.num_sms) grid = c.num_sms;
  CUtensorMap m[6];
  if (P) {
    g.x2 = w.a2; g.y2 = w.b2;
    g.pos = w.pos; g.wt = wt; g.wbar = w.wbar;
    g.gpos = w.gpos; g.rowsum = w.rowsum; g.pl = w.pl; g.nl = w.nl;
    g.dumpS = dumpS;
    g.out = w.GA;
    const long long rowsX = (long long)p.C * p.Cs * g.nblkD, rowsY = (long long)p.C * p.Ns * g.nblkD;
    const long long rowsYT = (long long)p.C * slab_blocks(p.Ns) * p.D;
    if (tc_make_map(&m[0], w.Ahi, rowsX, 32, kTileM) || tc_make_map(&m[1], w.Alo, rowsX, 32, kTileM) ||
        tc_make_map(&m[2], w.Bhi, rowsY, 32, g.N1) || tc_make_map(&m[3], w.Blo, rowsY, 32, g.N1) ||
        tc_make_map(&m[4], w.BhiT, rowsYT, 32, g.N2) || tc_make_map(&m[5], w.BloT, rowsYT, 32, g.N2))
      return KGE_ERR_CUDA;
    return launch_width(c, true, grid, smem, m, g);
  }
  g.Xhi = w.Bhi; g.Xlo = w.Blo;
  if (ent && ent->n_shards == 1 && neg_ids) { g.xids = neg_ids; g.xtab = *ent; }
  if (w.BnRaw) g.xraw = w.BnRaw;
  g.gsn = w.gsn;
  g.out = w.Bn;
  const long long rowsV = (long long)p.C * slab_blocks(p.Cs) * p.Ns, rowsA = (long long)p.C * slab_blocks(p.Cs) * p.D;
  if (tc_make_map(&m[0], w.VhiT, rowsV, 32, kTileM) || tc_make_map(&m[1], w.VloT, rowsV, 32, kTileM) ||
      tc_make_map(&m[2], w.AhiT, rowsA, 32, g.N1) || tc_make_map(&m[3], w.AloT, rowsA, 32, g.N1))
    return KGE_ERR_CUDA;
  return launch_width(c, false, grid, smem, m, g);
}

}
```

dgl-ke_b200/csrc/kge_rescal.cu:

```cuda
#include "kge_common.cuh"

namespace kge {


constexpr int kBlock = 256;
constexpr int kWarps = kBlock / 32;
constexpr int kMaxV = 4;

__global__ void __launch_bounds__(kBlock) k_rescal_fwd(StepParams p, const float* __restrict__ hbase,
                                                        const float* __restrict__ tbase, const float* __restrict__ rbase,
                                                        TableView ent, TableView rel, BatchView b, StepWs w,
                                                        bool dense, bool want_pos, bool want_a) {
  extern __shared__ __align__(16) float sm[];
  const int D = p.D;
  float* sh = sm;
  float* st = sm + D;
  float* sMh = sm + 2 * D;
  float* sMt = sm + 3 * D;
  __shared__ float red[kWarps];
  const long long i = blockIdx.x;
  const float *h, *t, *M;
  if (dense) {
    h = hbase + i * (long long)D; t = tbase + i * (long long)D; M = rbase + i * (long long)p.Dr;
    if (!want_pos) { if (p.neg_head) h = t; else t = h; }
  } else {
    h = node_row(p, ent, b, w, b.head_local[i]);
    t = node_row(p, ent, b, w, b.tail_local[i]);
    M = row_ptr(rel, b.rel_ids[i]);
  }
  for (int k = threadIdx.x; k < D; k += kBlock) { sh[k] = h[k]; st[k] = t[k]; }
  __syncthreads();
  const int warp = threadIdx.x >> 5, lane = threadIdx.x & 31, nv = D >> 2;
  const bool reg_on = (!dense) && (p.reg_coef > 0.f && p.reg_norm > 0);
  float reg = 0.f;
  for (int k = warp; k < D; k += kWarps) {
    const float* row = M + (long long)k * D;
    float ah = 0.f, at = 0.f;
    for (int v = lane; v < nv; v += 32) {
      float4 m4 = ld4_stream(row + 4 * v);
      ah += f4_dot(m4, ld4(sh + 4 * v));
      at += f4_dot(m4, ld4(st + 4 * v));
      if (reg_on) reg += abs_pow4_sum(m4, p.reg_norm);
    }
    ah = warp_sum(ah); at = warp_sum(at);
    if (lane == 0) { sMh[k] = ah; sMt[k] = at; }
  }
  __syncthreads();
  float pos = 0.f;
  for (int k = threadIdx.x; k < D; k += kBlock) {
    pos += sh[k] * sMt[k];
    if (want_a) {
      const float av = p.neg_head ? sMt[k] : sMh[k];
      if (w.Ahi) {
        float hh, ll;
        split_tf32(av, hh, ll);
        const long long o = slab_off(i / p.Cs, slab_blocks(D), p.Cs, (int)(i % p.Cs), k);
        w.Ahi[o] = hh; w.Alo[o] = ll;
        if (w.AhiT) {
          const long long ot = slabT_off(i / p.Cs, p.Cs, D, (int)(i % p.Cs), k);
          w.AhiT[ot] = hh; w.AloT[ot] = ll;
        }
      }
      else w.A[i * (long long)D + k] = av;
    }
    if (!dense) w.Mt[i * (long long)D + k] = sMt[k];
  }
  pos = warp_sum(pos); reg = warp_sum(reg);
  if (lane == 0) red[warp] = pos;
  __syncthreads();
  if (threadIdx.x == 0) {
    float s = 0.f;
    for (int q = 0; q < kWarps; ++q) s += red[q];
    if (want_pos) w.pos[i] = s;
  }
  __syncthreads();
  if (reg_on) {
    if (lane == 0) red[warp] = reg;
    __syncthreads();
    if (threadIdx.x == 0) {
      float s = 0.f;
      for (int q = 0; q < kWarps; ++q) s += red[q];
      w.regp[i] = s;
    }
  } else if (!dense && threadIdx.x == 0) {
    w.regp[i] = 0.f;
  }
}

int launch_rescal_prep(const LaunchCtx& c, const StepParams& p, const TableView& ent, const TableView& rel,
                       const BatchView& b, const StepWs& w) {
  size_t smem = 4 * (size_t)p.D * sizeof(float);
  KGE_LAUNCH(c, k_rescal_fwd, (unsigned)p.B, kBlock, smem, p, nullptr, nullptr, nullptr, ent, rel, b, w, false, true, true);
  return launch_prep_nonedge(c, p, ent, rel, b, w);
}

void launch_rescal_prep_dense(const LaunchCtx& c, const StepParams& p, const float* head, const float* relr,
                              const float* tail, const StepWs& w, bool want_pos, bool want_a) {
  size_t smem = 4 * (size_t)p.D * sizeof(float);
  TableView none{};
  BatchView nb{};
  KGE_LAUNCH(c, k_rescal_fwd, (unsigned)p.B, kBlock, smem, p, head, tail, relr, none, none, nb, w, true, want_pos, want_a);
}

__global__ void __launch_bounds__(kBlock) k_rescal_bwd(StepParams p, TableView ent, TableView rel, BatchView b, StepWs w) {
  extern __shared__ __align__(16) float sm[];
  const int D = p.D;
  float* sh = sm;
  float* st = sm + D;
  float* su = sm + 2 * D;
  float* sy = sm + 3 * D;
  __shared__ float red[kWarps];
  const long long i = blockIdx.x;
  const long long hl = b.head_local[i], tl = b.tail_local[i], rid = b.rel_ids[i];
  const float* h = node_row(p, ent, b, w, hl);
  const float* t = node_row(p, ent, b, w, tl);
  const float* M = row_ptr(rel, rid);
  float* GR = w.GR + i * (long long)p.Dr;
  const float g = w.gpos[i];
  const float* ga = w.GA + i * (long long)D;
  for (int k = threadIdx.x; k < D; k += kBlock) {
    float hk = h[k];
    sh[k] = hk; st[k] = t[k];
    su[k] = p.neg_head ? (ga[k] + g * hk) : ga[k];
    sy[k] = 0.f; sy[D + k] = 0.f;
  }
  __syncthreads();
  const int warp = threadIdx.x >> 5, lane = threadIdx.x & 31, nv = D >> 2;
  float4 y1[kMaxV], y2[kMaxV];
#pragma unroll
  for (int q = 0; q < kMaxV; ++q) { y1[q] = make_float4(0.f, 0.f, 0.f, 0.f); y2[q] = y1[q]; }
  float gs = 0.f;
  const float* pvec = p.neg_head ? st : sh;
  for (int k = warp; k < D; k += kWarps) {
    const float* row = M + (long long)k * D;
    const float uk = p.neg_head ? ga[k] : su[k];
    const float u1 = su[k], ghk = g * sh[k], hk = sh[k];
#pragma unroll
    for (int q = 0; q < kMaxV; ++q) {
      int v = lane + 32 * q;
      if (v < nv) {
        float4 m4 = ld4(row + 4 * v);
        float4 p4 = ld4(pvec + 4 * v), t4 = ld4(st + 4 * v);
        float4 dM = f4_add(f4_add(f4_scale(p4, uk), f4_scale(t4, ghk)), reg_grad4(m4, p.reg_norm, p.reg_coef));
        st4(GR + (long long)k * D + 4 * v, dM);
        gs += f4_dot(dM, dM);
        y1[q] = f4_fma(m4, u1, y1[q]);
        if (!p.neg_head) y2[q] = f4_fma(m4, hk, y2[q]);
      }
    }
  }
#pragma unroll
  for (int q = 0; q < kMaxV; ++q) {
    int v = lane + 32 * q;
    if (v < nv) {
      atomicAdd(&sy[4 * v + 0], y1[q].x); atomicAdd(&sy[4 * v + 1], y1[q].y);
      atomicAdd(&sy[4 * v + 2], y1[q].z); atomicAdd(&sy[4 * v + 3], y1[q].w);
      if (!p.neg_head) {
        atomicAdd(&sy[D + 4 * v + 0], y2[q].x); atomicAdd(&sy[D + 4 * v + 1], y2[q].y);
        atomicAdd(&sy[D + 4 * v + 2], y2[q].z); atomicAdd(&sy[D + 4 * v + 3], y2[q].w);
      }
    }
  }
  gs = warp_sum(gs);
  if (lane == 0) red[warp] = gs;
  __syncthreads();
  const float* mt = w.Mt + i * (long long)D;
  float* ngh = w.NG + hl * (long long)D;
  float* ngt = w.NG + tl * (long long)D;
  for (int k = threadIdx.x; k < D; k += kBlock) {
    float dh, dt;
    if (p.neg_head) { dt = sy[k]; dh = g * mt[k]; }
    else { dh = sy[k] + g * mt[k]; dt = g * sy[D + k]; }
    atomicAdd(ngh + k, dh);
    atomicAdd(ngt + k, dt);
  }
  if (threadIdx.x == 0) {
    float s = 0.f;
    for (int q = 0; q < kWarps; ++q) s += red[q];
    w.gsr[i] = s / (float)p.Dr;
  }
}

void launch_rescal_chain(const LaunchCtx& c, const StepParams& p, const TableView& ent, const TableView& rel,
                         const BatchView& b, const StepWs& w) {
  size_t smem = 5 * (size_t)p.D * sizeof(float);
  KGE_LAUNCH(c, k_rescal_bwd, (unsigned)p.B, kBlock, smem, p, ent, rel, b, w);
}

}
```

dgl-ke_b200/csrc/kge_rows.cu:

```cuda
#include "kge_common.cuh"

namespace kge {


constexpr int kRowBlock = 256;
constexpr int kWarpsPerBlock = kRowBlock / kWarp;

__global__ void __launch_bounds__(kRowBlock) k_gather(TableView t, const long long* __restrict__ idx,
                                                       long long n, float* __restrict__ out) {
  long long job = (long long)blockIdx.x * kWarpsPerBlock + (threadIdx.x >> 5);
  if (job >= n) return;
  int lane = threadIdx.x & 31;
  const float* src = row_ptr(t, idx[job]);
  float* dst = out + job * (long long)t.dim;
  int nv = t.dim >> 2;
  for (int v = lane; v < nv; v += kWarp) st4(dst + 4 * v, ld4_stream(src + 4 * v));
  for (int k = (nv << 2) + lane; k < t.dim; k += kWarp) dst[k] = src[k];
}

void launch_gather(const LaunchCtx& c, const TableView& t, const long long* idx, long long n, float* out) {
  if (n <= 0) return;
  KGE_LAUNCH(c, k_gather, ceil_div(n, kWarpsPerBlock), kRowBlock, 0, t, idx, n, out);
}

__global__ void k_fill_zero(float* p, long long n) {
  long long i = (long long)blockIdx.x * blockDim.x + threadIdx.x;
  long long stride = (long long)gridDim.x * blockDim.x;
  for (; i < n; i += stride) p[i] = 0.f;
}
void launch_fill_zero(const LaunchCtx& c, float* p, long long n) {
  if (n <= 0) return;
  int grid = (int)((n + 1023) / 1024);
  if (grid > c.num_sms * 8) grid = c.num_sms * 8;
  KGE_LAUNCH(c, k_fill_zero, grid, 256, 0, p, n);
}

struct EdgeAcc {
  float pos;
  float a2;
  float reg;
};

template <int MODEL>
__device__ __forceinline__ void edge_slice_real(float4 h, float4 r, float4 t, int neg_head, float4& a,
                                                EdgeAcc& acc) {
  if (MODEL == KGE_TRANSE_L1 || MODEL == KGE_TRANSE_L2) {
    float4 e = f4_sub(f4_add(h, r), t);
    if (MODEL == KGE_TRANSE_L2) acc.pos += f4_dot(e, e);
    else acc.pos += (fabsf(e.x) + fabsf(e.y)) + (fabsf(e.z) + fabsf(e.w));
    a = neg_head ? f4_sub(t, r) : f4_add(h, r);
    if (MODEL == KGE_TRANSE_L2) acc.a2 += f4_dot(a, a);
  } else {
    acc.pos += f4_hsum(f4_mul(f4_mul(h, r), t));
    a = neg_head ? f4_mul(t, r) : f4_mul(h, r);
  }
}

template <int MODEL>
__device__ __forceinline__ void edge_slice_cplx(float4 hr, float4 hi, float4 tr, float4 ti, float4 cr, float4 ci,
                                                int neg_head, float4& are, float4& aim, EdgeAcc& acc) {
  if (MODEL == KGE_COMPLEX) {
    float4 s = f4_sub(f4_add(f4_add(f4_mul(f4_mul(hr, tr), cr), f4_mul(f4_mul(hi, ti), cr)),
                             f4_mul(f4_mul(hr, ti), ci)),
                      f4_mul(f4_mul(hi, tr), ci));
    acc.pos += f4_hsum(s);
  } else {
    float4 dre = f4_sub(f4_sub(f4_mul(hr, cr), f4_mul(hi, ci)), tr);
    float4 dim = f4_sub(f4_add(f4_mul(hr, ci), f4_mul(hi, cr)), ti);
    acc.pos += (sqrtf(dre.x * dre.x + dim.x * dim.x) + sqrtf(dre.y * dre.y + dim.y * dim.y)) +
               (sqrtf(dre.z * dre.z + dim.z * dim.z) + sqrtf(dre.w * dre.w + dim.w * dim.w));
  }
  if (neg_head) {
    are = f4_add(f4_mul(tr, cr), f4_mul(ti, ci));
    aim = f4_add(f4_mul(f4_neg(tr), ci), f4_mul(ti, cr));
  } else {
    are = f4_sub(f4_mul(hr, cr), f4_mul(hi, ci));
    aim = f4_add(f4_mul(hr, ci), f4_mul(hi, cr));
  }
}

__device__ __forceinline__ void phase_cos_sin(float4 r, float inv_scale_den, float4& c, float4& s) {
  float p0 = r.x / inv_scale_den, p1 = r.y / inv_scale_den, p2 = r.z / inv_scale_den, p3 = r.w / inv_scale_den;
  sincosf(p0, &s.x, &c.x); sincosf(p1, &s.y, &c.y); sincosf(p2, &s.z, &c.z); sincosf(p3, &s.w, &c.w);
}

template <int MODEL, int KIT>
__device__ __forceinline__ void edge_forward(const StepParams& p, const float* __restrict__ h,
                                             const float* __restrict__ r, const float* __restrict__ t,
                                             const RowOut& a_out, int lane, float& pos_out, float& a2_out,
                                             float& reg_out, float& nrm_out, bool want_a) {
  EdgeAcc acc{0.f, 0.f, 0.f};
  const bool reg_on = (p.reg_coef > 0.f && p.reg_norm > 0);
  constexpr int kIt = KIT;
  constexpr int kItC = KIT > 1 ? KIT / 2 : 1;
  const float4 z4 = make_float4(0.f, 0.f, 0.f, 0.f);
  if (MODEL == KGE_COMPLEX || MODEL == KGE_ROTATE) {
    const int half = p.D >> 1, nvh = half >> 2;
    const float den = p.emb_init / 3.14159265358979323846f;
    for (int v0 = 0; v0 < nvh; v0 += kWarp * kItC) {
      float4 hr[kItC], hi[kItC], tr[kItC], ti[kItC], r0[kItC], r1[kItC];
#pragma unroll
      for (int it = 0; it < kItC; ++it) {
        const int v = v0 + lane + kWarp * it;
        const bool ok = v < nvh;
        hr[it] = ok ? ld4(h + 4 * v) : z4; hi[it] = ok ? ld4(h + half + 4 * v) : z4;
        tr[it] = ok ? ld4(t + 4 * v) : z4; ti[it] = ok ? ld4(t + half + 4 * v) : z4;
        r0[it] = ok ? ld4(r + 4 * v) : z4;
        r1[it] = (ok && MODEL == KGE_COMPLEX) ? ld4(r + half + 4 * v) : z4;
      }
#pragma unroll
      for (int it = 0; it < kItC; ++it) {
        const int v = v0 + lane + kWarp * it;
        if (v >= nvh) continue;
        float4 cr, ci;
        if (MODEL == KGE_COMPLEX) {
          cr = r0[it]; ci = r1[it];
          if (reg_on) acc.reg += abs_pow4_sum(cr, p.reg_norm) + abs_pow4_sum(ci, p.reg_norm);
        } else {
          if (reg_on) acc.reg += abs_pow4_sum(r0[it], p.reg_norm);
          phase_cos_sin(r0[it], den, cr, ci);
        }
        float4 are, aim;
        edge_slice_cplx<MODEL>(hr[it], hi[it], tr[it], ti[it], cr, ci, p.neg_head, are, aim, acc);
        if (want_a) { row_store4(a_out, 4 * v, are); row_store4(a_out, half + 4 * v, aim); }
      }
    }
  } else {
    const int nv = p.D >> 2;
    for (int v0 = 0; v0 < nv; v0 += kWarp * kIt) {
      float4 h4[kIt], r4[kIt], t4[kIt];
#pragma unroll
      for (int it = 0; it < kIt; ++it) {
        const int v = v0 + lane + kWarp * it;
        const bool ok = v < nv;
        h4[it] = ok ? ld4(h + 4 * v) : z4;
        r4[it] = ok ? ld4(r + 4 * v) : z4;
        t4[it] = ok ? ld4(t + 4 * v) : z4;
      }
#pragma unroll
      for (int it = 0; it < kIt; ++it) {
        const int v = v0 + lane + kWarp * it;
        if (v >= nv) continue;
        if (reg_on) acc.reg += abs_pow4_sum(r4[it], p.reg_norm);
        float4 a;
        edge_slice_real<MODEL>(h4[it], r4[it], t4[it], p.neg_head, a, acc);
        if (want_a) row_store4(a_out, 4 * v, a);
      }
    }
  }
  float s = warp_sum(acc.pos);
  a2_out = warp_sum(acc.a2);
  reg_out = warp_sum(acc.reg);
  nrm_out = 0.f;
  if (MODEL == KGE_TRANSE_L2) { nrm_out = sqrtf(s); pos_out = p.gamma - nrm_out; }
  else if (MODEL == KGE_TRANSE_L1 || MODEL == KGE_ROTATE) pos_out = p.gamma - s;
  else pos_out = s;
}

__host__ __device__ inline int prep_block_rows(const StepWs& w) { return (w.AhiT || w.BhiT) ? kPrepRows : kWarpsPerBlock; }

template <int MODEL, int KIT>
__global__ void __launch_bounds__(kRowBlock, 3) k_prep(StepParams p, TableView ent, TableView rel, BatchView b, StepWs w,
                                                        int blk0) {
  extern __shared__ float4 prep_stage_f4[];
  float* const stage = reinterpret_cast<float*>(prep_stage_f4);
  const int warp = threadIdx.x >> 5, lane = threadIdx.x & 31;
  const bool reg_on = (p.reg_coef > 0.f && p.reg_norm > 0);
  const int rows = prep_block_rows(w);
  const int eblk = (p.Cs + rows - 1) / rows;
  long long blk = (long long)blk0 + blockIdx.x;
  const bool edge = blk < (long long)p.C * eblk;
  if (!edge) blk -= (long long)p.C * eblk;
  const int R = edge ? p.Cs : p.Ns, nblk = edge ? eblk : (p.Ns + rows - 1) / rows;
  const long long chunk = blk / nblk;
  const int rb = (int)(blk % nblk);
  const int nrows = min(rows, R - rb * rows);
  float* const hiT = edge ? w.AhiT : w.BhiT;
  float* const loT = edge ? w.AloT : w.BloT;
  const int S = prep_stage_stride(p.D);

  for (int rl = warp; rl < nrows; rl += kWarpsPerBlock) {
    const int row = rb * rows + rl;
    float* const st = hiT ? stage + rl * S : nullptr;
    if (edge) {
      const long long job = chunk * p.Cs + row;
      const float* h = head_row(p, ent, b, w, job);
      const float* t = tail_row(p, ent, b, w, job);
      const float* r = row_ptr(rel, b.rel_ids[job]);
      float pos, a2, reg, nrm;
      const RowOut ao{w.Ahi ? nullptr : w.A + job * (long long)p.D, w.Ahi, w.Alo, chunk, slab_blocks(p.D), p.Cs, row, st};
      edge_forward<MODEL, 1>(p, h, r, t, ao, lane, pos, a2, reg, nrm, true);
      if (lane == 0) {
        w.pos[job] = pos;
        if (MODEL == KGE_TRANSE_L2) { w.a2[job] = a2; w.pnorm[job] = nrm; }
        w.regp[job] = reg;
      }
    } else {
      const long long job = chunk * p.Ns + row;
      const long long ro = job * (long long)p.D;
      const float* src = w.BnRaw ? w.BnRaw + ro : row_ptr(ent, b.neg_ids[job]);
      const RowOut bo{p.fused ? nullptr : w.Bn + ro, w.Bhi, w.Blo, chunk, slab_blocks(p.D), p.Ns, row, st};
      float b2 = 0.f, reg = 0.f;
      const int nv = p.D >> 2;
      for (int v0 = 0; v0 < nv; v0 += kWarp * KIT) {
        float4 x[KIT];
#pragma unroll
        for (int it = 0; it < KIT; ++it) {
          const int v = v0 + lane + kWarp * it;
          x[it] = (v < nv) ? ld4_stream(src + 4 * v) : make_float4(0.f, 0.f, 0.f, 0.f);
        }
#pragma unroll
        for (int it = 0; it < KIT; ++it) {
          const int v = v0 + lane + kWarp * it;
          if (v >= nv) continue;
          row_store4(bo, 4 * v, x[it]);
          if (MODEL == KGE_TRANSE_L2) b2 += f4_dot(x[it], x[it]);
          if (reg_on) reg += abs_pow4_sum(x[it], p.reg_norm);
        }
      }
      b2 = warp_sum(b2); reg = warp_sum(reg);
      if (lane == 0) {
        if (MODEL == KGE_TRANSE_L2) w.b2[job] = b2;
        w.regp[p.B + job] = reg;
      }
    }
  }
  if (!hiT) return;
  __syncthreads();
  if (lane >= nrows) return;
  const long long base = ((chunk * nblk + rb) * (long long)p.D) * 32 + lane;
  const float* srow = stage + lane * S;
  for (int g = warp; g < (p.D >> 2); g += kWarpsPerBlock) {
    float4 h, l;
    split_tf32_4(*reinterpret_cast<const float4*>(srow + 4 * g), h, l);
    float* dh = hiT + base + (long long)(4 * g) * 32;
    float* dl = loT + base + (long long)(4 * g) * 32;
    dh[0] = h.x; dh[32] = h.y; dh[64] = h.z; dh[96] = h.w;
    dl[0] = l.x; dl[32] = l.y; dl[64] = l.z; dl[96] = l.w;
  }
}

size_t prep_smem(const StepWs& w, int D) { return (w.AhiT || w.BhiT) ? prep_stage_bytes(D) : 0; }

int prep_launched(int D) {
  const cudaError_t e = cudaGetLastError();
  return e == cudaSuccess ? KGE_OK : fail(KGE_ERR_CUDA, "k_prep launch (d=%d): %s", D, cudaGetErrorString(e));
}

template <int KIT>
__global__ void __launch_bounds__(kRowBlock) k_gather_nodes(StepParams p, TableView ent, BatchView b, StepWs w) {
  const long long u = (long long)blockIdx.x * kWarpsPerBlock + (threadIdx.x >> 5);
  if (u >= node_count(p)) return;
  const int lane = threadIdx.x & 31;
  const bool reg_on = (p.reg_coef > 0.f && p.reg_norm > 0);
  const float* src = row_ptr(ent, b.node_ids[u]);
  float* dst = w.NC + u * (long long)p.D;
  const int nv = p.D >> 2;
  float reg = 0.f;
  for (int v0 = 0; v0 < nv; v0 += kWarp * KIT) {
    float4 x[KIT];
#pragma unroll
    for (int it = 0; it < KIT; ++it) {
      const int v = v0 + lane + kWarp * it;
      x[it] = (v < nv) ? ld4_stream(src + 4 * v) : make_float4(0.f, 0.f, 0.f, 0.f);
    }
#pragma unroll
    for (int it = 0; it < KIT; ++it) {
      const int v = v0 + lane + kWarp * it;
      if (v >= nv) continue;
      st4(dst + 4 * v, x[it]);
      if (reg_on) reg += abs_pow4_sum(x[it], p.reg_norm);
    }
  }
  reg = warp_sum(reg);
  if (lane == 0) w.regp[p.B + p.Nn + u] = reg;
}

void launch_gather_nodes(const LaunchCtx& c, const StepParams& p, const TableView& ent, const BatchView& b,
                         const StepWs& w) {
  if (ent.n_shards > 1) KGE_LAUNCH(c, k_gather_nodes<4>, ceil_div(p.U, kWarpsPerBlock), kRowBlock, 0, p, ent, b, w);
  else KGE_LAUNCH(c, k_gather_nodes<2>, ceil_div(p.U, kWarpsPerBlock), kRowBlock, 0, p, ent, b, w);
}

template <int MODEL>
__global__ void __launch_bounds__(kRowBlock) k_prep_dense(StepParams p, const float* __restrict__ head,
                                                           const float* __restrict__ relr,
                                                           const float* __restrict__ tail,
                                                           const float* __restrict__ negrows, StepWs w,
                                                           bool want_pos, bool want_a) {
  long long job = (long long)blockIdx.x * kWarpsPerBlock + (threadIdx.x >> 5);
  const int lane = threadIdx.x & 31;
  if (job < p.B) {
    float pos, a2, reg, nrm;
    const float* hrow = head + job * (long long)p.D;
    const float* trow = tail + job * (long long)p.D;
    if (!want_pos) { if (p.neg_head) hrow = trow; else trow = hrow; }
    const long long ro = job * (long long)p.D;
    const RowOut ao{(want_a && !w.Ahi) ? w.A + ro : nullptr, want_a ? w.Ahi : nullptr, want_a ? w.Alo : nullptr,
                    job / p.Cs, slab_blocks(p.D), p.Cs, (int)(job % p.Cs), nullptr};
    edge_forward<MODEL, 1>(p, hrow, relr + job * (long long)p.Dr, trow, ao, lane, pos, a2, reg, nrm, want_a);
    if (lane == 0) {
      if (want_pos) w.pos[job] = pos;
      if (want_a && MODEL == KGE_TRANSE_L2) w.a2[job] = a2;
    }
    return;
  }
  job -= p.B;
  if (job < p.Nn && negrows != nullptr) {
    const float* src = negrows + job * (long long)p.D;
    const long long ro = job * (long long)p.D;
    const RowOut bo{nullptr, w.Bhi, w.Blo, job / p.Ns, slab_blocks(p.D), p.Ns, (int)(job % p.Ns), nullptr};
    float b2 = 0.f;
    for (int v = lane; v < (p.D >> 2); v += kWarp) {
      float4 x = ld4(src + 4 * v);
      b2 += f4_dot(x, x);
      row_store4(bo, 4 * v, x);
    }
    b2 = warp_sum(b2);
    if (lane == 0 && MODEL == KGE_TRANSE_L2) w.b2[job] = b2;
  }
}

#define KGE_DISPATCH_MODEL(model, ...)                                      \
  switch (model) {                                                          \
    case KGE_TRANSE_L1: { constexpr int M = KGE_TRANSE_L1; __VA_ARGS__; } break; \
    case KGE_TRANSE_L2: { constexpr int M = KGE_TRANSE_L2; __VA_ARGS__; } break; \
    case KGE_DISTMULT:  { constexpr int M = KGE_DISTMULT;  __VA_ARGS__; } break; \
    case KGE_COMPLEX:   { constexpr int M = KGE_COMPLEX;   __VA_ARGS__; } break; \
    case KGE_ROTATE:    { constexpr int M = KGE_ROTATE;    __VA_ARGS__; } break; \
    default: break;                                                         \
  }

int launch_prep(const LaunchCtx& c, const StepParams& p, const TableView& ent, const TableView& rel,
                const BatchView& b, const StepWs& w) {
  const int rows = prep_block_rows(w);
  const int blocks = p.C * (ceil_div(p.Cs, rows) + ceil_div(p.Ns, rows));
  const size_t smem = prep_smem(w, p.D);
  int rc = KGE_OK;
  if (ent.n_shards > 1) {
    KGE_DISPATCH_MODEL(p.model, if (!(rc = smem_optin((const void*)k_prep<M, 4>, smem)))
                                  KGE_LAUNCH(c, (k_prep<M, 4>), blocks, kRowBlock, smem, p, ent, rel, b, w, 0));
  } else {
    KGE_DISPATCH_MODEL(p.model, if (!(rc = smem_optin((const void*)k_prep<M, 1>, smem)))
                                  KGE_LAUNCH(c, (k_prep<M, 1>), blocks, kRowBlock, smem, p, ent, rel, b, w, 0));
  }
  return rc ? rc : prep_launched(p.D);
}

int launch_prep_nonedge(const LaunchCtx& c, const StepParams& p, const TableView& ent, const TableView& rel,
                        const BatchView& b, const StepWs& w) {
  const size_t smem = prep_smem(w, p.D);
  if (int rc = smem_optin((const void*)k_prep<KGE_DISTMULT, 1>, smem)) return rc;
  const int rows = prep_block_rows(w);
  KGE_LAUNCH(c, (k_prep<KGE_DISTMULT, 1>), p.C * ceil_div(p.Ns, rows), kRowBlock, smem, p, ent, rel, b, w,
             p.C * ceil_div(p.Cs, rows));
  return prep_launched(p.D);
}

void launch_prep_dense(const LaunchCtx& c, const StepParams& p, const float* head, const float* relr,
                       const float* tail, const float* negrows, const StepWs& w, bool want_pos, bool want_a) {
  long long jobs = p.B + ((negrows && (p.model == KGE_TRANSE_L2 || w.Bhi)) ? p.Nn : 0);
  KGE_DISPATCH_MODEL(p.model, KGE_LAUNCH(c, k_prep_dense<M>, ceil_div(jobs, kWarpsPerBlock), kRowBlock, 0, p, head,
                                         relr, tail, negrows, w, want_pos, want_a));
}

struct LossRow {
  float w_i, inv2B, T, mx, den, uni;
  int adversarial, l2;
  int hinge, pairwise;
  float margin, ps, invBN;
};
__device__ __forceinline__ float crit(const LossRow& r, float x, float label, float& dx) {
  if (r.hinge) {
    const float t = r.margin - label * x;
    dx = (t < 0.f) ? 0.f : -label;
    return fmaxf(t, 0.f);
  }
  dx = -label * sigmoidf(-label * x);
  return softplusf(-label * x);
}
__device__ __forceinline__ float loss_elem(const LossRow& r, float sc, float dist, float& nls, float& rs, float& gp) {
  float g;
  if (r.pairwise) {
    float dd;
    const float l = crit(r, r.ps - sc, 1.f, dd);
    nls += l * r.w_i * r.uni;
    g = -dd * r.w_i * r.invBN;
    gp += dd * r.w_i * r.invBN;
  } else {
    const float pij = r.adversarial ? expf(sc * r.T - r.mx) / r.den : r.uni;
    float dd;
    const float l = crit(r, sc, -1.f, dd);
    nls += pij * (l * r.w_i);
    g = pij * dd * r.w_i * r.inv2B;
  }
  float coef = g;
  if (r.l2) { coef = (dist > 1.5e-15f) ? g / dist : 0.f; rs += coef; }
  return coef;
}

__global__ void __launch_bounds__(kRowBlock) k_loss(StepParams p, const float* __restrict__ pos,
                                                     const float* __restrict__ S, const float* __restrict__ wt,
                                                     const float* __restrict__ wbar, float* __restrict__ V,
                                                     float* __restrict__ gpos, float* __restrict__ rowsum,
                                                     float* __restrict__ pl, float* __restrict__ nl,
                                                     float* __restrict__ Vhi, float* __restrict__ Vlo,
                                                     float* __restrict__ VhiT, float* __restrict__ VloT) {
  long long i = (long long)blockIdx.x * kWarpsPerBlock + (threadIdx.x >> 5);
  if (i >= p.B) return;
  const int lane = threadIdx.x & 31;
  const float* s = S + i * (long long)p.Ns;
  float* v = V + i * (long long)p.Ns;
  LossRow r;
  r.w_i = wt ? wt[i] : 1.f;
  r.inv2B = 0.5f / (float)p.B;
  r.T = p.adv_temperature; r.mx = -INFINITY; r.den = 1.f; r.uni = 1.f / (float)p.Ns;
  r.adversarial = p.adversarial && !p.pairwise; r.l2 = (p.model == KGE_TRANSE_L2);
  r.hinge = p.hinge; r.pairwise = p.pairwise; r.margin = p.margin;
  r.ps = pos[i]; r.invBN = 1.f / ((float)p.B * (float)p.Ns);
  float gp = 0.f;
  const long long chunk = i / p.Cs;
  const int il = (int)(i % p.Cs), nblk = slab_blocks(p.Ns);
  float nls = 0.f, rs = 0.f;
  if (p.Ns <= 8 * kWarp) {
    float sc[8], ds[8];
#pragma unroll
    for (int q = 0; q < 8; ++q) {
      const int j = lane + kWarp * q;
      sc[q] = (j < p.Ns) ? s[j] : -INFINITY;
      ds[q] = (r.l2 && j < p.Ns) ? v[j] : 1.f;
    }
    if (r.adversarial) {
      float mx = -INFINITY;
#pragma unroll
      for (int q = 0; q < 8; ++q) mx = fmaxf(mx, sc[q] * r.T);
      r.mx = warp_max(mx);
      float d = 0.f;
#pragma unroll
      for (int q = 0; q < 8; ++q) if (lane + kWarp * q < p.Ns) d += expf(sc[q] * r.T - r.mx);
      r.den = warp_sum(d);
    }
#pragma unroll
    for (int q = 0; q < 8; ++q) {
      const int j = lane + kWarp * q;
      if (j >= p.Ns) continue;
      const float coef = loss_elem(r, sc[q], ds[q], nls, rs, gp);
      v[j] = coef;
      if (Vhi) {
        float hh, ll;
        split_tf32(coef, hh, ll);
        const long long o = slab_off(chunk, nblk, p.Cs, il, j);
        Vhi[o] = hh; Vlo[o] = ll;
        const long long ot = slabT_off(chunk, p.Cs, p.Ns, il, j);
        VhiT[ot] = hh; VloT[ot] = ll;
      }
    }
  } else {
    if (r.adversarial) {
      float mx = -INFINITY;
      for (int j = lane; j < p.Ns; j += kWarp) mx = fmaxf(mx, s[j] * r.T);
      r.mx = warp_max(mx);
      float d = 0.f;
      for (int j = lane; j < p.Ns; j += kWarp) d += expf(s[j] * r.T - r.mx);
      r.den = warp_sum(d);
    }
    for (int j = lane; j < p.Ns; j += kWarp) {
      const float coef = loss_elem(r, s[j], r.l2 ? v[j] : 1.f, nls, rs, gp);
      v[j] = coef;
      if (Vhi) {
        float hh, ll;
        split_tf32(coef, hh, ll);
        const long long o = slab_off(chunk, nblk, p.Cs, il, j);
        Vhi[o] = hh; Vlo[o] = ll;
        const long long ot = slabT_off(chunk, p.Cs, p.Ns, il, j);
        VhiT[ot] = hh; VloT[ot] = ll;
      }
    }
  }
  nls = warp_sum(nls);
  rs = warp_sum(rs);
  gp = warp_sum(gp);
  if (lane == 0) {
    float ps = pos[i];
    float wb = wt ? *wbar : 1.f;
    if (p.pairwise) {
      pl[i] = 0.f;
      gpos[i] = gp;
    } else {
      float dd;
      pl[i] = crit(r, ps, 1.f, dd);
      gpos[i] = dd * wb * r.inv2B;
    }
    nl[i] = nls;
// ... 648 lines not shown
```

dgl-ke_b200/csrc/kge_tc.cuh:

```cuda
#pragma once
#include <cuda.h>
#include <cuda_runtime.h>
#include <stdint.h>

namespace kge {
namespace tc {

__device__ __forceinline__ uint32_t smem_u32(const void* p) { return (uint32_t)__cvta_generic_to_shared(p); }

__device__ __forceinline__ bool elect_one() {
  uint32_t pred = 0;
  asm volatile(
      "{\n\t.reg .pred P1;\n\t"
      "elect.sync _|P1, 0xFFFFFFFF;\n\t"
      "selp.b32 %0, 1, 0, P1;\n\t}"
      : "=r"(pred));
  return pred != 0;
}

__device__ __forceinline__ void mbar_init(uint64_t* bar, uint32_t count) {
  asm volatile("mbarrier.init.shared::cta.b64 [%0], %1;" ::"r"(smem_u32(bar)), "r"(count));
}
__device__ __forceinline__ void mbar_expect_tx(uint64_t* bar, uint32_t bytes) {
  asm volatile("mbarrier.arrive.expect_tx.shared::cta.b64 _, [%0], %1;" ::"r"(smem_u32(bar)), "r"(bytes) : "memory");
}
__device__ __forceinline__ void mbar_arrive(uint64_t* bar) {
  asm volatile("mbarrier.arrive.shared::cta.b64 _, [%0];" ::"r"(smem_u32(bar)) : "memory");
}
__device__ __forceinline__ void mbar_wait(uint64_t* bar, uint32_t parity) {
  uint32_t done;
  do {
    asm volatile(
        "{\n\t.reg .pred p;\n\t"
        "mbarrier.try_wait.parity.shared::cta.b64 p, [%1], %2;\n\t"
        "selp.u32 %0, 1, 0, p;\n\t}"
        : "=r"(done) : "r"(smem_u32(bar)), "r"(parity) : "memory");
  } while (!done);
}
__device__ __forceinline__ void tma_load_2d(void* dst, const CUtensorMap* map, uint64_t* bar, int x, int y) {
  asm volatile(
      "cp.async.bulk.tensor.2d.shared::cluster.global.mbarrier::complete_tx::bytes [%0], [%1, {%3, %4}], [%2];"
      ::"r"(smem_u32(dst)), "l"(map), "r"(smem_u32(bar)), "r"(x), "r"(y) : "memory");
}
__device__ __forceinline__ void bulk_g2s(void* dst, const void* src, uint32_t bytes, uint64_t* bar) {
  asm volatile("cp.async.bulk.shared::cluster.global.mbarrier::complete_tx::bytes [%0], [%1], %2, [%3];"
               ::"r"(smem_u32(dst)), "l"(src), "r"(bytes), "r"(smem_u32(bar)) : "memory");
}
__device__ __forceinline__ void bulk_s2g(void* dst, const void* src, uint32_t bytes) {
  asm volatile("cp.async.bulk.global.shared::cta.bulk_group [%0], [%1], %2;"
               ::"l"(dst), "r"(smem_u32(src)), "r"(bytes) : "memory");
}
__device__ __forceinline__ void bulk_commit() { asm volatile("cp.async.bulk.commit_group;" ::: "memory"); }
template <int N>
__device__ __forceinline__ void bulk_wait_read() { asm volatile("cp.async.bulk.wait_group.read %0;" ::"n"(N) : "memory"); }
__device__ __forceinline__ void bulk_wait_all() { asm volatile("cp.async.bulk.wait_group 0;" ::: "memory"); }
__device__ __forceinline__ void tma_prefetch_desc(const CUtensorMap* map) {
  asm volatile("prefetch.tensormap [%0];" ::"l"(map) : "memory");
}
__device__ __forceinline__ void wgmma_fence() { asm volatile("wgmma.fence.sync.aligned;" ::: "memory"); }
__device__ __forceinline__ void wgmma_commit() { asm volatile("wgmma.commit_group.sync.aligned;" ::: "memory"); }
template <int N>
__device__ __forceinline__ void wgmma_wait() { asm volatile("wgmma.wait_group.sync.aligned %0;" ::"n"(N) : "memory"); }
template <int N>
__device__ __forceinline__ void reg_fence(float (&d)[N]) {
#pragma unroll
  for (int i = 0; i < N; ++i) asm volatile("" : "+f"(d[i])::"memory");
}
__device__ __forceinline__ void reg_fence(uint32_t (&a)[4]) {
  asm volatile("" : "+r"(a[0]), "+r"(a[1]), "+r"(a[2]), "+r"(a[3])::"memory");
}
#define KGE_D4(i) "+f"(d[i]), "+f"(d[i + 1]), "+f"(d[i + 2]), "+f"(d[i + 3])
#define KGE_D16(i) KGE_D4(i), KGE_D4(i + 4), KGE_D4(i + 8), KGE_D4(i + 12)
#define KGE_D32(i) KGE_D16(i), KGE_D16(i + 16)
template <int N>
__device__ __forceinline__ void wgmma_ss(float (&d)[N / 2], uint64_t adesc, uint64_t bdesc, uint32_t accumulate);
template <int N>
__device__ __forceinline__ void wgmma_rs(float (&d)[N / 2], const uint32_t (&a)[4], uint64_t bdesc, uint32_t accumulate);
template <>
__device__ __forceinline__ void wgmma_ss<64>(float (&d)[32], uint64_t adesc, uint64_t bdesc, uint32_t accumulate) {
  asm volatile("{\n\t.reg .pred p;\n\tsetp.ne.b32 p, %34, 0;\n\t"
               "wgmma.mma_async.sync.aligned.m64n64k8.f32.tf32.tf32 {%0,%1,%2,%3,%4,%5,%6,%7,%8,%9,%10,%11,%12,%13,%14,%15,%16,%17,%18,%19,%20,%21,%22,%23,%24,%25,%26,%27,%28,%29,%30,%31}, %32, %33, p, 1, 1;\n\t}"
               : KGE_D32(0)
               : "l"(adesc), "l"(bdesc), "r"(accumulate));
}
template <>
__device__ __forceinline__ void wgmma_ss<128>(float (&d)[64], uint64_t adesc, uint64_t bdesc, uint32_t accumulate) {
  asm volatile("{\n\t.reg .pred p;\n\tsetp.ne.b32 p, %66, 0;\n\t"
               "wgmma.mma_async.sync.aligned.m64n128k8.f32.tf32.tf32 {%0,%1,%2,%3,%4,%5,%6,%7,%8,%9,%10,%11,%12,%13,%14,%15,%16,%17,%18,%19,%20,%21,%22,%23,%24,%25,%26,%27,%28,%29,%30,%31,%32,%33,%34,%35,%36,%37,%38,%39,%40,%41,%42,%43,%44,%45,%46,%47,%48,%49,%50,%51,%52,%53,%54,%55,%56,%57,%58,%59,%60,%61,%62,%63}, %64, %65, p, 1, 1;\n\t}"
               : KGE_D32(0), KGE_D32(32)
               : "l"(adesc), "l"(bdesc), "r"(accumulate));
}
template <>
__device__ __forceinline__ void wgmma_ss<200>(float (&d)[100], uint64_t adesc, uint64_t bdesc, uint32_t accumulate) {
  asm volatile("{\n\t.reg .pred p;\n\tsetp.ne.b32 p, %102, 0;\n\t"
               "wgmma.mma_async.sync.aligned.m64n200k8.f32.tf32.tf32 {%0,%1,%2,%3,%4,%5,%6,%7,%8,%9,%10,%11,%12,%13,%14,%15,%16,%17,%18,%19,%20,%21,%22,%23,%24,%25,%26,%27,%28,%29,%30,%31,%32,%33,%34,%35,%36,%37,%38,%39,%40,%41,%42,%43,%44,%45,%46,%47,%48,%49,%50,%51,%52,%53,%54,%55,%56,%57,%58,%59,%60,%61,%62,%63,%64,%65,%66,%67,%68,%69,%70,%71,%72,%73,%74,%75,%76,%77,%78,%79,%80,%81,%82,%83,%84,%85,%86,%87,%88,%89,%90,%91,%92,%93,%94,%95,%96,%97,%98,%99}, %100, %101, p, 1, 1;\n\t}"
               : KGE_D32(0), KGE_D32(32), KGE_D32(64), KGE_D4(96)
               : "l"(adesc), "l"(bdesc), "r"(accumulate));
}
template <>
__device__ __forceinline__ void wgmma_ss<208>(float (&d)[104], uint64_t adesc, uint64_t bdesc, uint32_t accumulate) {
  asm volatile("{\n\t.reg .pred p;\n\tsetp.ne.b32 p, %106, 0;\n\t"
               "wgmma.mma_async.sync.aligned.m64n208k8.f32.tf32.tf32 {%0,%1,%2,%3,%4,%5,%6,%7,%8,%9,%10,%11,%12,%13,%14,%15,%16,%17,%18,%19,%20,%21,%22,%23,%24,%25,%26,%27,%28,%29,%30,%31,%32,%33,%34,%35,%36,%37,%38,%39,%40,%41,%42,%43,%44,%45,%46,%47,%48,%49,%50,%51,%52,%53,%54,%55,%56,%57,%58,%59,%60,%61,%62,%63,%64,%65,%66,%67,%68,%69,%70,%71,%72,%73,%74,%75,%76,%77,%78,%79,%80,%81,%82,%83,%84,%85,%86,%87,%88,%89,%90,%91,%92,%93,%94,%95,%96,%97,%98,%99,%100,%101,%102,%103}, %104, %105, p, 1, 1;\n\t}"
               : KGE_D32(0), KGE_D32(32), KGE_D32(64), KGE_D4(96), KGE_D4(100)
               : "l"(adesc), "l"(bdesc), "r"(accumulate));
}
template <>
__device__ __forceinline__ void wgmma_ss<256>(float (&d)[128], uint64_t adesc, uint64_t bdesc, uint32_t accumulate) {
  asm volatile("{\n\t.reg .pred p;\n\tsetp.ne.b32 p, %130, 0;\n\t"
               "wgmma.mma_async.sync.aligned.m64n256k8.f32.tf32.tf32 {%0,%1,%2,%3,%4,%5,%6,%7,%8,%9,%10,%11,%12,%13,%14,%15,%16,%17,%18,%19,%20,%21,%22,%23,%24,%25,%26,%27,%28,%29,%30,%31,%32,%33,%34,%35,%36,%37,%38,%39,%40,%41,%42,%43,%44,%45,%46,%47,%48,%49,%50,%51,%52,%53,%54,%55,%56,%57,%58,%59,%60,%61,%62,%63,%64,%65,%66,%67,%68,%69,%70,%71,%72,%73,%74,%75,%76,%77,%78,%79,%80,%81,%82,%83,%84,%85,%86,%87,%88,%89,%90,%91,%92,%93,%94,%95,%96,%97,%98,%99,%100,%101,%102,%103,%104,%105,%106,%107,%108,%109,%110,%111,%112,%113,%114,%115,%116,%117,%118,%119,%120,%121,%122,%123,%124,%125,%126,%127}, %128, %129, p, 1, 1;\n\t}"
               : KGE_D32(0), KGE_D32(32), KGE_D32(64), KGE_D32(96)
               : "l"(adesc), "l"(bdesc), "r"(accumulate));
}
template <>
__device__ __forceinline__ void wgmma_rs<128>(float (&d)[64], const uint32_t (&a)[4], uint64_t bdesc, uint32_t accumulate) {
  asm volatile("{\n\t.reg .pred p;\n\tsetp.ne.b32 p, %69, 0;\n\t"
               "wgmma.mma_async.sync.aligned.m64n128k8.f32.tf32.tf32 {%0,%1,%2,%3,%4,%5,%6,%7,%8,%9,%10,%11,%12,%13,%14,%15,%16,%17,%18,%19,%20,%21,%22,%23,%24,%25,%26,%27,%28,%29,%30,%31,%32,%33,%34,%35,%36,%37,%38,%39,%40,%41,%42,%43,%44,%45,%46,%47,%48,%49,%50,%51,%52,%53,%54,%55,%56,%57,%58,%59,%60,%61,%62,%63}, {%64,%65,%66,%67}, %68, p, 1, 1;\n\t}"
               : KGE_D32(0), KGE_D32(32)
               : "r"(a[0]), "r"(a[1]), "r"(a[2]), "r"(a[3]), "l"(bdesc), "r"(accumulate));
}
template <>
__device__ __forceinline__ void wgmma_rs<200>(float (&d)[100], const uint32_t (&a)[4], uint64_t bdesc, uint32_t accumulate) {
  asm volatile("{\n\t.reg .pred p;\n\tsetp.ne.b32 p, %105, 0;\n\t"
               "wgmma.mma_async.sync.aligned.m64n200k8.f32.tf32.tf32 {%0,%1,%2,%3,%4,%5,%6,%7,%8,%9,%10,%11,%12,%13,%14,%15,%16,%17,%18,%19,%20,%21,%22,%23,%24,%25,%26,%27,%28,%29,%30,%31,%32,%33,%34,%35,%36,%37,%38,%39,%40,%41,%42,%43,%44,%45,%46,%47,%48,%49,%50,%51,%52,%53,%54,%55,%56,%57,%58,%59,%60,%61,%62,%63,%64,%65,%66,%67,%68,%69,%70,%71,%72,%73,%74,%75,%76,%77,%78,%79,%80,%81,%82,%83,%84,%85,%86,%87,%88,%89,%90,%91,%92,%93,%94,%95,%96,%97,%98,%99}, {%100,%101,%102,%103}, %104, p, 1, 1;\n\t}"
               : KGE_D32(0), KGE_D32(32), KGE_D32(64), KGE_D4(96)
               : "r"(a[0]), "r"(a[1]), "r"(a[2]), "r"(a[3]), "l"(bdesc), "r"(accumulate));
}
#undef KGE_D4
#undef KGE_D16
#undef KGE_D32

__device__ __forceinline__ uint64_t make_desc(uint32_t saddr) {
  uint64_t d = 0;
  d |= (uint64_t)((saddr >> 4) & 0x3FFF);
  d |= (uint64_t)1 << 16;
  d |= (uint64_t)(1024 >> 4) << 32;
  d |= (uint64_t)1 << 62;
  return d;
}

__device__ __forceinline__ float ex2a(float x) { float y; asm("ex2.approx.ftz.f32 %0, %1;" : "=f"(y) : "f"(x)); return y; }
__device__ __forceinline__ float lg2a(float x) { float y; asm("lg2.approx.ftz.f32 %0, %1;" : "=f"(y) : "f"(x)); return y; }
__device__ __forceinline__ float rcpa(float x) { float y; asm("rcp.approx.ftz.f32 %0, %1;" : "=f"(y) : "f"(x)); return y; }
__device__ __forceinline__ float rsqrta(float x) { float y; asm("rsqrt.approx.ftz.f32 %0, %1;" : "=f"(y) : "f"(x)); return y; }
__device__ __forceinline__ float sqrta(float x) { float y; asm("sqrt.approx.ftz.f32 %0, %1;" : "=f"(y) : "f"(x)); return y; }

}

int tc_make_map(CUtensorMap* m, const float* base, long long rows, long long cols, int box_rows);

}
```

Baseline: 30.88 million.

## Feed wgmma A operand from registers with on-the-fly 3xTF32 split in fused kernels

```diff
diff --git a/dgl-ke_b200/csrc/kge_abi.cu b/dgl-ke_b200/csrc/kge_abi.cu
--- a/dgl-ke_b200/csrc/kge_abi.cu
+++ b/dgl-ke_b200/csrc/kge_abi.cu
@@ -273,6 +273,7 @@
   const size_t B = (size_t)p.B, Nn = (size_t)p.Nn, U = (size_t)(p.U > 0 ? p.U : 0);
   const bool um = !opt.force_tiles && use_umma(h, p);
   const bool fused = p.fused != 0;
+  const FusedHilo hl = fused ? fused_hilo(p) : FusedHilo{false, false};
   const size_t sA = B * slab_blocks(p.D) * 32 + 8192, sB = Nn * slab_blocks(p.D) * 32 + 8192;
   const size_t sV = B * slab_blocks(p.Ns) * 32 + 8192;
   const size_t sAT = (size_t)p.C * slab_blocks(p.Cs) * p.D * 32 + 8192, sBT = (size_t)p.C * slab_blocks(p.Ns) * p.D * 32 + 8192;
@@ -286,10 +287,11 @@
       {&w->rowsum, B, true}, {&w->colsum, Nn, true}, {&w->pl, B, true}, {&w->nl, B, true}, {&w->wbar, 4, true},
       {&w->gsr, B, true}, {&w->gsn, Nn, true}, {&w->colpart, (size_t)ceil_div(p.Cs, 128) * Nn, fused},
       {&w->Mt, BD, p.model == KGE_RESCAL},
-      {&w->Ahi, sA, um}, {&w->Alo, sA, um}, {&w->Bhi, sB, um}, {&w->Blo, sB, um},
+      {&w->Ahi, sA, um && (!fused || hl.a)}, {&w->Alo, sA, um && (!fused || hl.a)}, {&w->Af, sA, fused && !hl.a},
+      {&w->Bhi, sB, um}, {&w->Blo, sB, um},
       {&w->Vhi, sV, um && !fused}, {&w->Vlo, sV, um && !fused},
       {&w->AhiT, sAT, um}, {&w->AloT, sAT, um}, {&w->BhiT, sBT, um}, {&w->BloT, sBT, um},
-      {&w->VhiT, sVT, um}, {&w->VloT, sVT, um},
+      {&w->VhiT, sVT, um && (!fused || hl.v)}, {&w->VloT, sVT, um && (!fused || hl.v)}, {&w->VT, sVT, fused},
       {&w->NC, U * p.D, p.use_nc != 0},
       {&w->regp, B + Nn + (U ? 2 * B : 0), true},
   };
diff --git a/dgl-ke_b200/csrc/kge_common.cuh b/dgl-ke_b200/csrc/kge_common.cuh
--- a/dgl-ke_b200/csrc/kge_common.cuh
+++ b/dgl-ke_b200/csrc/kge_common.cuh
@@ -90,6 +90,8 @@
   float *AhiT, *AloT;
   float *BhiT, *BloT;
   float *VhiT, *VloT;
+  float* Af;
+  float* VT;
 };
 
 struct BatchView {
@@ -205,15 +207,19 @@
   long long chunk;
   int nblk, R, row;
   float* stage;
+  float* slab;
 };
 __device__ __forceinline__ void row_store4(const RowOut& o, int col, float4 v) {
   if (o.f32) *reinterpret_cast<float4*>(o.f32 + col) = v;
-  if (o.hi) {
-    float4 h, l;
-    split_tf32_4(v, h, l);
+  if (o.hi || o.slab) {
     const long long off = slab_off(o.chunk, o.nblk, o.R, o.row, col);
-    *reinterpret_cast<float4*>(o.hi + off) = h;
-    *reinterpret_cast<float4*>(o.lo + off) = l;
+    if (o.slab) *reinterpret_cast<float4*>(o.slab + off) = v;
+    if (o.hi) {
+      float4 h, l;
+      split_tf32_4(v, h, l);
+      *reinterpret_cast<float4*>(o.hi + off) = h;
+      *reinterpret_cast<float4*>(o.lo + off) = l;
+    }
   }
   if (o.stage) *reinterpret_cast<float4*>(o.stage + col) = v;
 }
@@ -377,6 +383,8 @@
 };
 bool fused_supported(const StepParams&);
 int fused_prefetch_slots(const StepParams& p, int mode);
+struct FusedHilo { bool a, v; };
+FusedHilo fused_hilo(const StepParams& p);
 int fused_launch(const LaunchCtx&, const StepParams&, const StepWs&, int mode, const float* wt, float* dumpS, float* dumpV,
                  const TableView* ent, const long long* neg_ids, const FusedPrefetch* pf);
 
diff --git a/dgl-ke_b200/csrc/kge_fused.cu b/dgl-ke_b200/csrc/kge_fused.cu
--- a/dgl-ke_b200/csrc/kge_fused.cu
+++ b/dgl-ke_b200/csrc/kge_fused.cu
@@ -33,6 +33,7 @@
   int nblkD;
   int nS1, nS2;
   uint32_t stage1Bytes, stage2Bytes;
+  float* VT;
   float *VhiT, *VloT;
   float* colpart;
   int ncolpart;
@@ -119,6 +120,8 @@
   __syncwarp();
 }
 
+__host__ __device__ constexpr bool k_reg_a(int n) { return n < 256; }
+
 template <int NW, int KS>
 __device__ __forceinline__ void kblock_3xtf32(float (&acc)[NW / 2], uint64_t dXh, uint64_t dXl, uint64_t dYh, uint64_t dYl) {
   wgmma_fence();
@@ -132,6 +135,48 @@
   wgmma_commit();
 }
 
+__device__ __forceinline__ float lds_f32(uint32_t a) {
+  float v;
+  asm volatile("ld.shared.f32 %0, [%1];" : "=f"(v) : "r"(a) : "memory");
+  return v;
+}
+
+__device__ __forceinline__ void a_frag(uint32_t row, int ks, int g, int q, uint32_t (&ah)[4], uint32_t (&al)[4]) {
+  const uint32_t c0 = row + (uint32_t)(((((2 * ks) ^ g) << 2) + q) << 2);
+  const uint32_t c1 = row + (uint32_t)(((((2 * ks + 1) ^ g) << 2) + q) << 2);
+  const float a[4] = {lds_f32(c0), lds_f32(c0 + 1024u), lds_f32(c1), lds_f32(c1 + 1024u)};
+#pragma unroll
+  for (int r = 0; r < 4; ++r) {
+    float hi, lo;
+    split_tf32(a[r], hi, lo);
+    ah[r] = __float_as_uint(hi); al[r] = __float_as_uint(lo);
+  }
+}
+
+template <int N>
+__device__ __forceinline__ void kstep_rs(float (&acc)[N / 2], const uint32_t (&ah)[4], const uint32_t (&al)[4],
+                                         uint64_t dYh, uint64_t dYl) {
+  wgmma_fence();
+  wgmma_rs<N>(acc, ah, dYh, 1u);
+  wgmma_rs<N>(acc, ah, dYl, 1u);
+  wgmma_rs<N>(acc, al, dYh, 1u);
+  wgmma_commit();
+}
+
+template <int N, int KS>
+__device__ __forceinline__ void kblock_rs(float (&acc)[N / 2], uint32_t (&ah)[2][4], uint32_t (&al)[2][4], uint32_t row,
+                                          int g, int q, uint64_t dYh, uint64_t dYl, uint64_t* release, int lane) {
+#pragma unroll
+  for (int ks = 0; ks < KS; ++ks) {
+    a_frag(row, ks, g, q, ah[ks & 1], al[ks & 1]);
+    const uint64_t o = (uint64_t)(ks * 2);
+    kstep_rs<N>(acc, ah[ks & 1], al[ks & 1], dYh + o, dYl + o);
+    wgmma_wait<1>();
+    reg_fence(ah[(ks + 1) & 1]); reg_fence(al[(ks + 1) & 1]);
+    if (ks == 0 && release && lane == 0) mbar_arrive(release);
+  }
+}
+
 template <int NV>
 __device__ __forceinline__ int vsm_idx(int i, int k) {
   const int g = i & 7, h = (i >> 3) & 1, kk = k & 7;
@@ -150,11 +195,7 @@
     split_tf32(a[r], hi, lo);
     ah[r] = __float_as_uint(hi); al[r] = __float_as_uint(lo);
   }
-  wgmma_fence();
-  wgmma_rs<NW>(acc2, ah, dYh, 1u);
-  wgmma_rs<NW>(acc2, ah, dYl, 1u);
-  wgmma_rs<NW>(acc2, al, dYh, 1u);
-  wgmma_commit();
+  kstep_rs<NW>(acc2, ah, al, dYh, dYl);
 }
 
 __device__ __forceinline__ int tile_row() {
@@ -165,7 +206,7 @@
 
 template <int NV, int NW>
 __global__ void __launch_bounds__(kThreadsF, 1)
-k_fused_pos(const __grid_constant__ CUtensorMap mXh, const __grid_constant__ CUtensorMap mXl,
+k_fused_pos(const __grid_constant__ CUtensorMap mX, const __grid_constant__ CUtensorMap mXl,
             const __grid_constant__ CUtensorMap mYh1, const __grid_constant__ CUtensorMap mYl1,
             const __grid_constant__ CUtensorMap mYh2, const __grid_constant__ CUtensorMap mYl2, FusedArgs g) {
   extern __shared__ __align__(1024) uint8_t smem_raw[];
@@ -187,6 +228,7 @@
   const int nkb2 = (g.Ry + 31) >> 5;
   const int nchunks = (g.D + NW - 1) / NW;
   constexpr uint32_t yBytes1 = (uint32_t)NV * 128u;
+  constexpr uint32_t xBytes1 = k_reg_a(NV) ? 16384u : 32768u;
   constexpr uint32_t yBytes2 = (uint32_t)NW * 128u;
   const bool l2 = g.model == KGE_TRANSE_L2;
   const int nhand = g.pf_slots > 0 ? 1 : 3;
@@ -200,8 +242,8 @@
     asm volatile("fence.mbarrier_init.release.cluster;" ::: "memory");
   }
   if (warp == kProducerWarp && lane == 0) {
-    tma_prefetch_desc(&mXh); tma_prefetch_desc(&mXl); tma_prefetch_desc(&mYh1);
-    tma_prefetch_desc(&mYl1); tma_prefetch_desc(&mYh2); tma_prefetch_desc(&mYl2);
+    tma_prefetch_desc(&mX); if (!k_reg_a(NV)) tma_prefetch_desc(&mXl); tma_prefetch_desc(&mYh1); tma_prefetch_desc(&mYl1);
+    tma_prefetch_desc(&mYh2); tma_prefetch_desc(&mYl2);
   }
   __syncthreads();
 
@@ -219,11 +261,11 @@
         const int yx = (c * g.nblkD + kb) * g.Rx + m0;
         const int yy = (c * g.nblkD + kb) * g.Ry;
         if (elect_one()) {
-          mbar_expect_tx(&full1[s], 2u * 16384u + 2u * yBytes1);
-          tma_load_2d(st, &mXh, &full1[s], 0, yx);
-          tma_load_2d(st + 16384, &mXl, &full1[s], 0, yx);
-          tma_load_2d(st + 32768, &mYh1, &full1[s], 0, yy);
-          tma_load_2d(st + 32768 + yBytes1, &mYl1, &full1[s], 0, yy);
+          mbar_expect_tx(&full1[s], xBytes1 + 2u * yBytes1);
+          tma_load_2d(st, &mX, &full1[s], 0, yx);
+          if (!k_reg_a(NV)) tma_load_2d(st + 16384, &mXl, &full1[s], 0, yx);
+          tma_load_2d(st + xBytes1, &mYh1, &full1[s], 0, yy);
+          tma_load_2d(st + xBytes1 + yBytes1, &mYl1, &full1[s], 0, yy);
         }
         __syncwarp();
       }
@@ -263,10 +305,14 @@
         for (int b = 0; b < kTileM / 32; ++b) {
           const int i = 32 * b + lane;
           if (i < rows) {
-            float hi, lo;
-            split_tf32(v[b], hi, lo);
             const long long o = slabT_off(c, g.Rx, g.Ry, m0 + i, j);
-            g.VhiT[o] = hi; g.VloT[o] = lo;
+            if (g.VhiT) {
+              float hi, lo;
+              split_tf32(v[b], hi, lo);
+              g.VhiT[o] = hi; g.VloT[o] = lo;
+            } else {
+              g.VT[o] = v[b];
+            }
           }
           s += v[b];
         }
@@ -285,7 +331,7 @@
   }
   } else {
     asm volatile("setmaxnreg.inc.sync.aligned.u32 224;");
-    const int wg = warp >> 2, q = lane & 3;
+    const int q = lane & 3;
     const int et = threadIdx.x;
     uint32_t n1 = 0, n2 = 0;
     for (int tile = blockIdx.x; tile < ntiles; tile += gridDim.x) {
@@ -301,26 +347,50 @@
       float acc[NV / 2];
 #pragma unroll
       for (int i = 0; i < NV / 2; ++i) acc[i] = 0.f;
-      for (int kb = 0; kb < nkb1; ++kb, ++n1) {
-        const uint32_t s = n1 % g.nS1;
-        mbar_wait(&full1[s], (n1 / g.nS1) & 1);
-        const uint32_t st = smem_u32(ring + (size_t)s * g.stage1Bytes);
-        const uint64_t dXh = make_desc(st + wg * 8192u), dXl = make_desc(st + 16384u + wg * 8192u);
-        const uint64_t dYh = make_desc(st + 32768u), dYl = make_desc(st + 32768u + yBytes1);
-        const int kleft = g.D - kb * 32;
-        const int ksteps = kleft >= 32 ? 4 : (kleft >> 3);
-        switch (ksteps) {
-          case 4: kblock_3xtf32<NV, 4>(acc, dXh, dXl, dYh, dYl); break;
-          case 3: kblock_3xtf32<NV, 3>(acc, dXh, dXl, dYh, dYl); break;
-          case 2: kblock_3xtf32<NV, 2>(acc, dXh, dXl, dYh, dYl); break;
-          default: kblock_3xtf32<NV, 1>(acc, dXh, dXl, dYh, dYl); break;
-        }
-        if (kb > 0) {
-          wgmma_wait<1>();
-          if (lane == 0) mbar_arrive(&empty1[(n1 - 1) % g.nS1]);
-        }
-      }
-      wgmma_wait<0>();
+      if constexpr (k_reg_a(NV)) {
+        uint32_t ah[2][4], al[2][4];
+        const int g8 = (lane >> 2);
+        for (int kb = 0; kb < nkb1; ++kb, ++n1) {
+          const uint32_t s = n1 % g.nS1;
+          mbar_wait(&full1[s], (n1 / g.nS1) & 1);
+          const uint32_t st = smem_u32(ring + (size_t)s * g.stage1Bytes);
+          const uint32_t xrow = st + (uint32_t)(16 * warp + g8) * 128u;
+          const uint64_t dYh = make_desc(st + xBytes1), dYl = make_desc(st + xBytes1 + yBytes1);
+          const int kleft = g.D - kb * 32;
+          const int ksteps = kleft >= 32 ? 4 : (kleft >> 3);
+          uint64_t* rel = kb > 0 ? &empty1[(n1 - 1) % g.nS1] : nullptr;
+          switch (ksteps) {
+            case 4: kblock_rs<NV, 4>(acc, ah, al, xrow, g8, q, dYh, dYl, rel, lane); break;
+            case 3: kblock_rs<NV, 3>(acc, ah, al, xrow, g8, q, dYh, dYl, rel, lane); break;
+            case 2: kblock_rs<NV, 2>(acc, ah, al, xrow, g8, q, dYh, dYl, rel, lane); break;
+            default: kblock_rs<NV, 1>(acc, ah, al, xrow, g8, q, dYh, dYl, rel, lane); break;
+          }
+        }
+        wgmma_wait<0>();
+        reg_fence(ah[0]); reg_fence(ah[1]); reg_fence(al[0]); reg_fence(al[1]);
+      } else {
+        const int wg = warp >> 2;
+        for (int kb = 0; kb < nkb1; ++kb, ++n1) {
+          const uint32_t s = n1 % g.nS1;
+          mbar_wait(&full1[s], (n1 / g.nS1) & 1);
+          const uint32_t st = smem_u32(ring + (size_t)s * g.stage1Bytes);
+          const uint64_t dXh = make_desc(st + wg * 8192u), dXl = make_desc(st + 16384u + wg * 8192u);
+          const uint64_t dYh = make_desc(st + xBytes1), dYl = make_desc(st + xBytes1 + yBytes1);
+          const int kleft = g.D - kb * 32;
+          const int ksteps = kleft >= 32 ? 4 : (kleft >> 3);
+          switch (ksteps) {
+            case 4: kblock_3xtf32<NV, 4>(acc, dXh, dXl, dYh, dYl); break;
+            case 3: kblock_3xtf32<NV, 3>(acc, dXh, dXl, dYh, dYl); break;
+            case 2: kblock_3xtf32<NV, 2>(acc, dXh, dXl, dYh, dYl); break;
+            default: kblock_3xtf32<NV, 1>(acc, dXh, dXl, dYh, dYl); break;
+          }
+          if (kb > 0) {
+            wgmma_wait<1>();
+            if (lane == 0) mbar_arrive(&empty1[(n1 - 1) % g.nS1]);
+          }
+        }
+        wgmma_wait<0>();
+      }
       if (lane == 0) mbar_arrive(&empty1[(n1 - 1) % g.nS1]);
       reg_fence(acc);
       epi_bar();
@@ -472,7 +542,7 @@
 
 template <int NW, bool FLAT>
 __global__ void __launch_bounds__(kThreadsF, 1)
-k_fused_neg(const __grid_constant__ CUtensorMap mVh, const __grid_constant__ CUtensorMap mVl,
+k_fused_neg(const __grid_constant__ CUtensorMap mV, const __grid_constant__ CUtensorMap mVl,
             const __grid_constant__ CUtensorMap mAh, const __grid_constant__ CUtensorMap mAl, FusedArgs g) {
   extern __shared__ __align__(1024) uint8_t smem_raw[];
   __shared__ __align__(8) uint64_t full[kMaxS1], empty[kMaxS1];
@@ -487,6 +557,7 @@
   const int nch = (g.D + NW - 1) / NW;
   constexpr uint32_t aBytes = (uint32_t)kTileM * 128u;
   constexpr uint32_t bBytes = (uint32_t)NW * 128u;
+  constexpr uint32_t vBytes = k_reg_a(NW) ? aBytes : 2u * aBytes;
   const bool l2 = g.model == KGE_TRANSE_L2;
 
   if (threadIdx.x == 0) {
@@ -495,7 +566,7 @@
     asm volatile("fence.mbarrier_init.release.cluster;" ::: "memory");
   }
   if (warp == kProducerWarp && lane == 0) {
-    tma_prefetch_desc(&mVh); tma_prefetch_desc(&mVl); tma_prefetch_desc(&mAh); tma_prefetch_desc(&mAl);
+    tma_prefetch_desc(&mV); if (!k_reg_a(NW)) tma_prefetch_desc(&mVl); tma_prefetch_desc(&mAh); tma_prefetch_desc(&mAl);
   }
   __syncthreads();
 
@@ -513,11 +584,11 @@
           const int yv = (c * nkb + kb) * g.Rx + m0;
           const int ya = (c * nkb + kb) * g.D + ch * NW;
           if (elect_one()) {
-            mbar_expect_tx(&full[s], 2u * aBytes + 2u * bBytes);
-            tma_load_2d(st, &mVh, &full[s], 0, yv);
-            tma_load_2d(st + aBytes, &mVl, &full[s], 0, yv);
-            tma_load_2d(st + 2 * aBytes, &mAh, &full[s], 0, ya);
-            tma_load_2d(st + 2 * aBytes + bBytes, &mAl, &full[s], 0, ya);
+            mbar_expect_tx(&full[s], vBytes + 2u * bBytes);
+            tma_load_2d(st, &mV, &full[s], 0, yv);
+            if (!k_reg_a(NW)) tma_load_2d(st + aBytes, &mVl, &full[s], 0, yv);
+            tma_load_2d(st + vBytes, &mAh, &full[s], 0, ya);
+            tma_load_2d(st + vBytes + bBytes, &mAl, &full[s], 0, ya);
           }
           __syncwarp();
         }
@@ -539,7 +610,10 @@
           const int j = m0 + e / g.Ry, i = e % g.Ry;
           if (j >= g.Rx) break;
           const long long o = slabT_off(c, g.Ry, g.Rx, i, j);
-          g.dumpV[((long long)c * g.Rx + j) * g.Ry + i] = g.VhiT[o] + g.VloT[o];
+          float hi, lo;
+          if (k_reg_a(NW)) split_tf32(g.VT[o], hi, lo);
+          else { hi = g.VhiT[o]; lo = g.VloT[o]; }
+          g.dumpV[((long long)c * g.Rx + j) * g.Ry + i] = hi + lo;
         }
       }
       float cs[2] = {0.f, 0.f};
@@ -589,27 +663,50 @@
         float acc[NW / 2];
 #pragma unroll
         for (int i = 0; i < NW / 2; ++i) acc[i] = 0.f;
-        for (int kb = 0; kb < nkb; ++kb, ++n) {
-          const uint32_t s = n % g.nS1;
-          mbar_wait(&full[s], (n / g.nS1) & 1);
-          const uint32_t st = smem_u32(ring + (size_t)s * g.stage1Bytes);
-          const uint64_t dVh = make_desc(st + wg * 8192u), dVl = make_desc(st + aBytes + wg * 8192u);
-          const uint64_t dAh = make_desc(st + 2 * aBytes), dAl = make_desc(st + 2 * aBytes + bBytes);
-          const int kleft = g.Ry - kb * 32;
-          const int ksteps = kleft >= 32 ? 4 : (kleft >> 3);
-          switch (ksteps) {
-            case 4: kblock_3xtf32<NW, 4>(acc, dVh, dVl, dAh, dAl); break;
-            case 3: kblock_3xtf32<NW, 3>(acc, dVh, dVl, dAh, dAl); break;
-            case 2: kblock_3xtf32<NW, 2>(acc, dVh, dVl, dAh, dAl); break;
-            default: kblock_3xtf32<NW, 1>(acc, dVh, dVl, dAh, dAl); break;
-          }
-          if (kb > 0) {
-            wgmma_wait<1>();
-            if (lane == 0) mbar_arrive(&empty[(n - 1) % g.nS1]);
-          }
-        }
-        if (early) load_b(0, d0, 0);
-        wgmma_wait<0>();
+        if constexpr (k_reg_a(NW)) {
+          uint32_t ah[2][4], al[2][4];
+          for (int kb = 0; kb < nkb; ++kb, ++n) {
+            const uint32_t s = n % g.nS1;
+            mbar_wait(&full[s], (n / g.nS1) & 1);
+            const uint32_t st = smem_u32(ring + (size_t)s * g.stage1Bytes);
+            const uint32_t vrow = st + (uint32_t)(16 * warp + (lane >> 2)) * 128u;
+            const uint64_t dAh = make_desc(st + vBytes), dAl = make_desc(st + vBytes + bBytes);
+            const int kleft = g.Ry - kb * 32;
+            const int ksteps = kleft >= 32 ? 4 : (kleft >> 3);
+            uint64_t* rel = kb > 0 ? &empty[(n - 1) % g.nS1] : nullptr;
+            switch (ksteps) {
+              case 4: kblock_rs<NW, 4>(acc, ah, al, vrow, lane >> 2, q, dAh, dAl, rel, lane); break;
+              case 3: kblock_rs<NW, 3>(acc, ah, al, vrow, lane >> 2, q, dAh, dAl, rel, lane); break;
+              case 2: kblock_rs<NW, 2>(acc, ah, al, vrow, lane >> 2, q, dAh, dAl, rel, lane); break;
+              default: kblock_rs<NW, 1>(acc, ah, al, vrow, lane >> 2, q, dAh, dAl, rel, lane); break;
+            }
+          }
+          if (early) load_b(0, d0, 0);
+          wgmma_wait<0>();
+          reg_fence(ah[0]); reg_fence(ah[1]); reg_fence(al[0]); reg_fence(al[1]);
+        } else {
+          for (int kb = 0; kb < nkb; ++kb, ++n) {
+            const uint32_t s = n % g.nS1;
+            mbar_wait(&full[s], (n / g.nS1) & 1);
+            const uint32_t st = smem_u32(ring + (size_t)s * g.stage1Bytes);
+            const uint64_t dVh = make_desc(st + wg * 8192u), dVl = make_desc(st + aBytes + wg * 8192u);
+            const uint64_t dAh = make_desc(st + vBytes), dAl = make_desc(st + vBytes + bBytes);
+            const int kleft = g.Ry - kb * 32;
+            const int ksteps = kleft >= 32 ? 4 : (kleft >> 3);
+            switch (ksteps) {
+              case 4: kblock_3xtf32<NW, 4>(acc, dVh, dVl, dAh, dAl); break;
+              case 3: kblock_3xtf32<NW, 3>(acc, dVh, dVl, dAh, dAl); break;
+              case 2: kblock_3xtf32<NW, 2>(acc, dVh, dVl, dAh, dAl); break;
+              default: kblock_3xtf32<NW, 1>(acc, dVh, dVl, dAh, dAl); break;
+            }
+            if (kb > 0) {
+              wgmma_wait<1>();
+              if (lane == 0) mbar_arrive(&empty[(n - 1) % g.nS1]);
+            }
+          }
+          if (early) load_b(0, d0, 0);
+          wgmma_wait<0>();
+        }
         if (lane == 0) mbar_arrive(&empty[(n - 1) % g.nS1]);
         reg_fence(acc);
 #pragma unroll
@@ -654,6 +751,8 @@
 }
 
 namespace {
+constexpr uint32_t kLoBytes = (uint32_t)kTileM * 128u;
+uint32_t stage1_bytes(int n) { return (k_reg_a(n) ? 1u : 2u) * kLoBytes + 2u * (uint32_t)n * 128u; }
 struct Geometry { int Rx, Ry, N1, N2, nS1, nS2, pf_slots; uint32_t ringBytes, stage1Bytes, stage2Bytes, pf_off; bool ok; };
 
 int neg_chunk_width(int D, bool want_prefetch) {
@@ -675,16 +774,17 @@
     q.Rx = p.Ns; q.Ry = p.Cs;
     q.ringBytes = kRingBytes;
     q.N1 = neg_chunk_width(p.D, want_prefetch);
-    q.stage1Bytes = 2u * kTileM * 128u + 2u * (uint32_t)q.N1 * 128u;
+    q.stage1Bytes = stage1_bytes(q.N1);
     q.nS1 = (int)(kRingBytes / q.stage1Bytes); if (q.nS1 > kMaxS1) q.nS1 = kMaxS1;
     q.ok = q.nS1 >= 2;
     if (q.ok && want_prefetch) {
-      int nS = q.nS1;
-      while (nS > 2 && kRingBytes - (uint32_t)nS * q.stage1Bytes < 2u * kMaxPf * row) --nS;
-      const uint32_t used = (uint32_t)nS * q.stage1Bytes;
+      const uint32_t fp = stage1_bytes(q.N1) + (k_reg_a(q.N1) ? kLoBytes : 0u);
+      int nS = (int)(kRingBytes / fp); if (nS > kMaxS1) nS = kMaxS1;
+      while (nS > 2 && kRingBytes - (uint32_t)nS * fp < 2u * kMaxPf * row) --nS;
+      const uint32_t used = (uint32_t)nS * fp;
       int slots = (int)((kRingBytes - used) / (2u * row));
       if (slots > kMaxPf) slots = kMaxPf;
-      if (slots >= 2) { q.pf_slots = slots; q.nS1 = nS; q.pf_off = used; }
+      if (slots >= 2 && nS >= 2) { q.pf_slots = slots; q.nS1 = nS; q.pf_off = used; }
     }
     return q;
   }
@@ -692,8 +792,9 @@
   q.N1 = q.Ry <= 64 ? 64 : (q.Ry <= 128 ? 128 : (q.Ry <= 208 ? 208 : 256));
   const uint32_t ring = want_prefetch ? kRingBytes : kRingBytesP;
   q.ringBytes = ring;
-  q.stage1Bytes = 2u * 16384u + 2u * (uint32_t)q.N1 * 128u;
-  int nS1 = (int)(ring / q.stage1Bytes); if (nS1 > kMaxS1) nS1 = kMaxS1;
+  q.stage1Bytes = stage1_bytes(q.N1);
+  const uint32_t fp1 = (want_prefetch && k_reg_a(q.N1)) ? q.stage1Bytes + kLoBytes : q.stage1Bytes;
+  int nS1 = (int)(ring / fp1); if (nS1 > kMaxS1) nS1 = kMaxS1;
   if (nS1 < 2) return q;
   const uint32_t vBytes = (uint32_t)q.N1 * 512u;
   const bool w200 = (p.D + 199) / 200 * 200 < (p.D + 127) / 128 * 128;
@@ -711,9 +812,9 @@
     if (!first.ok) first = t;
     const uint32_t want = 2u * kMaxPf * row;
     int s1 = t.nS1, s2 = t.nS2;
-    while (s1 > 2 && ring - (uint32_t)s1 * q.stage1Bytes < want) --s1;
+    while (s1 > 2 && ring - (uint32_t)s1 * fp1 < want) --s1;
     while (s2 > 2 && ring - (vBytes + (uint32_t)s2 * t.stage2Bytes) < want) --s2;
-    uint32_t used = (uint32_t)s1 * q.stage1Bytes;
+    uint32_t used = (uint32_t)s1 * fp1;
     if (vBytes + (uint32_t)s2 * t.stage2Bytes > used) used = vBytes + (uint32_t)s2 * t.stage2Bytes;
     int slots = (int)((ring - used) / (2u * row));
     if (slots > kMaxPf) slots = kMaxPf;
@@ -757,7 +858,10 @@
 template <int NW, bool FLAT>
 int launch_neg_src(const LaunchCtx& c, int grid, size_t smem, const CUtensorMap* m, const FusedArgs& g) {
   if (int rc = smem_optin((const void*)k_fused_neg<NW, FLAT>, smem)) return rc;
-  KGE_LAUNCH_NAMED(c, "k_fused<N: G_neg=V^T.A, mean sq>", (k_fused_neg<NW, FLAT>), grid, kThreadsF, smem, m[0], m[1], m[2], m[3], g);
+  static char name[64];
+  static std::once_flag once;
+  std::call_once(once, [] { snprintf(name, sizeof(name), "k_fused<N: G_neg=V^T.A, mean sq> NW=%d", NW); });
+  KGE_LAUNCH_NAMED(c, name, (k_fused_neg<NW, FLAT>), grid, kThreadsF, smem, m[0], m[1], m[2], m[3], g);
   return launch_error();
 }
 template <int NW>
@@ -776,6 +880,10 @@
 }
 
 int fused_prefetch_slots(const StepParams& p, int mode) { return geometry(p, mode, true).pf_slots; }
+
+FusedHilo fused_hilo(const StepParams& p) {
+  return FusedHilo{!k_reg_a(geometry(p, 0, false).N1), !k_reg_a(neg_chunk_width(p.D, false))};
+}
 
 int fused_launch(const LaunchCtx& c, const StepParams& p, const StepWs& w, int mode, const float* wt, float* dumpS,
                  float* dumpV, const TableView* ent, const long long* neg_ids, const FusedPrefetch* pf) {
@@ -797,7 +905,9 @@
     g.pf_neg_ids = pf->neg_ids; g.pf_nc = pf->nc; g.pf_bn = pf->bn;
     g.xtab = *ent;
   }
-  g.VhiT = w.VhiT; g.VloT = w.VloT; g.colpart = w.colpart; g.ncolpart = (p.Cs + kTileM - 1) / kTileM;
+  if (k_reg_a(geometry(p, 1, pf != nullptr && ent != nullptr).N1)) g.VT = w.VT;
+  else { g.VhiT = w.VhiT; g.VloT = w.VloT; }
+  g.colpart = w.colpart; g.ncolpart = (p.Cs + kTileM - 1) / kTileM;
   g.dumpV = dumpV;
   const size_t smem = q.ringBytes + 1024;
   const int mtiles = (g.Rx + kTileM - 1) / kTileM;
@@ -812,7 +922,8 @@
     g.out = w.GA;
     const long long rowsX = (long long)p.C * p.Cs * g.nblkD, rowsY = (long long)p.C * p.Ns * g.nblkD;
     const long long rowsYT = (long long)p.C * slab_blocks(p.Ns) * p.D;
-    if (tc_make_map(&m[0], w.Ahi, rowsX, 32, kTileM) || tc_make_map(&m[1], w.Alo, rowsX, 32, kTileM) ||
+    const bool ra = k_reg_a(g.N1);
+    if (tc_make_map(&m[0], ra ? w.Af : w.Ahi, rowsX, 32, kTileM) || tc_make_map(&m[1], ra ? w.Af : w.Alo, rowsX, 32, kTileM) ||
         tc_make_map(&m[2], w.Bhi, rowsY, 32, g.N1) || tc_make_map(&m[3], w.Blo, rowsY, 32, g.N1) ||
         tc_make_map(&m[4], w.BhiT, rowsYT, 32, g.N2) || tc_make_map(&m[5], w.BloT, rowsYT, 32, g.N2))
       return KGE_ERR_CUDA;
@@ -824,7 +935,8 @@
   g.gsn = w.gsn;
   g.out = w.Bn;
   const long long rowsV = (long long)p.C * slab_blocks(p.Cs) * p.Ns, rowsA = (long long)p.C * slab_blocks(p.Cs) * p.D;
-  if (tc_make_map(&m[0], w.VhiT, rowsV, 32, kTileM) || tc_make_map(&m[1], w.VloT, rowsV, 32, kTileM) ||
+  const bool rv = k_reg_a(g.N1);
+  if (tc_make_map(&m[0], rv ? w.VT : w.VhiT, rowsV, 32, kTileM) || tc_make_map(&m[1], rv ? w.VT : w.VloT, rowsV, 32, kTileM) ||
       tc_make_map(&m[2], w.AhiT, rowsA, 32, g.N1) || tc_make_map(&m[3], w.AloT, rowsA, 32, g.N1))
     return KGE_ERR_CUDA;
   return launch_width(c, false, grid, smem, m, g);
diff --git a/dgl-ke_b200/csrc/kge_rescal.cu b/dgl-ke_b200/csrc/kge_rescal.cu
--- a/dgl-ke_b200/csrc/kge_rescal.cu
+++ b/dgl-ke_b200/csrc/kge_rescal.cu
@@ -51,11 +51,12 @@
     pos += sh[k] * sMt[k];
     if (want_a) {
       const float av = p.neg_head ? sMt[k] : sMh[k];
-      if (w.Ahi) {
+      if (w.Ahi || w.Af) {
         float hh, ll;
         split_tf32(av, hh, ll);
         const long long o = slab_off(i / p.Cs, slab_blocks(D), p.Cs, (int)(i % p.Cs), k);
-        w.Ahi[o] = hh; w.Alo[o] = ll;
+        if (w.Af) w.Af[o] = av;
+        else { w.Ahi[o] = hh; w.Alo[o] = ll; }
         if (w.AhiT) {
           const long long ot = slabT_off(i / p.Cs, p.Cs, D, (int)(i % p.Cs), k);
           w.AhiT[ot] = hh; w.AloT[ot] = ll;
diff --git a/dgl-ke_b200/csrc/kge_rows.cu b/dgl-ke_b200/csrc/kge_rows.cu
--- a/dgl-ke_b200/csrc/kge_rows.cu
+++ b/dgl-ke_b200/csrc/kge_rows.cu
@@ -188,7 +188,8 @@
       const float* t = tail_row(p, ent, b, w, job);
       const float* r = row_ptr(rel, b.rel_ids[job]);
       float pos, a2, reg, nrm;
-      const RowOut ao{w.Ahi ? nullptr : w.A + job * (long long)p.D, w.Ahi, w.Alo, chunk, slab_blocks(p.D), p.Cs, row, st};
+      const RowOut ao{(w.Ahi || w.Af) ? nullptr : w.A + job * (long long)p.D, w.Ahi, w.Alo, chunk, slab_blocks(p.D), p.Cs,
+                      row, st, w.Af};
       edge_forward<MODEL, 1>(p, h, r, t, ao, lane, pos, a2, reg, nrm, true);
       if (lane == 0) {
         w.pos[job] = pos;
diff --git a/dgl-ke_b200/csrc/kge_tc.cuh b/dgl-ke_b200/csrc/kge_tc.cuh
--- a/dgl-ke_b200/csrc/kge_tc.cuh
+++ b/dgl-ke_b200/csrc/kge_tc.cuh
@@ -112,6 +112,13 @@
                : "l"(adesc), "l"(bdesc), "r"(accumulate));
 }
 template <>
+__device__ __forceinline__ void wgmma_rs<64>(float (&d)[32], const uint32_t (&a)[4], uint64_t bdesc, uint32_t accumulate) {
+  asm volatile("{\n\t.reg .pred p;\n\tsetp.ne.b32 p, %37, 0;\n\t"
+               "wgmma.mma_async.sync.aligned.m64n64k8.f32.tf32.tf32 {%0,%1,%2,%3,%4,%5,%6,%7,%8,%9,%10,%11,%12,%13,%14,%15,%16,%17,%18,%19,%20,%21,%22,%23,%24,%25,%26,%27,%28,%29,%30,%31}, {%32,%33,%34,%35}, %36, p, 1, 1;\n\t}"
+               : KGE_D32(0)
+               : "r"(a[0]), "r"(a[1]), "r"(a[2]), "r"(a[3]), "l"(bdesc), "r"(accumulate));
+}
+template <>
 __device__ __forceinline__ void wgmma_rs<128>(float (&d)[64], const uint32_t (&a)[4], uint64_t bdesc, uint32_t accumulate) {
   asm volatile("{\n\t.reg .pred p;\n\tsetp.ne.b32 p, %69, 0;\n\t"
                "wgmma.mma_async.sync.aligned.m64n128k8.f32.tf32.tf32 {%0,%1,%2,%3,%4,%5,%6,%7,%8,%9,%10,%11,%12,%13,%14,%15,%16,%17,%18,%19,%20,%21,%22,%23,%24,%25,%26,%27,%28,%29,%30,%31,%32,%33,%34,%35,%36,%37,%38,%39,%40,%41,%42,%43,%44,%45,%46,%47,%48,%49,%50,%51,%52,%53,%54,%55,%56,%57,%58,%59,%60,%61,%62,%63}, {%64,%65,%66,%67}, %68, p, 1, 1;\n\t}"
@@ -123,6 +130,20 @@
   asm volatile("{\n\t.reg .pred p;\n\tsetp.ne.b32 p, %105, 0;\n\t"
                "wgmma.mma_async.sync.aligned.m64n200k8.f32.tf32.tf32 {%0,%1,%2,%3,%4,%5,%6,%7,%8,%9,%10,%11,%12,%13,%14,%15,%16,%17,%18,%19,%20,%21,%22,%23,%24,%25,%26,%27,%28,%29,%30,%31,%32,%33,%34,%35,%36,%37,%38,%39,%40,%41,%42,%43,%44,%45,%46,%47,%48,%49,%50,%51,%52,%53,%54,%55,%56,%57,%58,%59,%60,%61,%62,%63,%64,%65,%66,%67,%68,%69,%70,%71,%72,%73,%74,%75,%76,%77,%78,%79,%80,%81,%82,%83,%84,%85,%86,%87,%88,%89,%90,%91,%92,%93,%94,%95,%96,%97,%98,%99}, {%100,%101,%102,%103}, %104, p, 1, 1;\n\t}"
                : KGE_D32(0), KGE_D32(32), KGE_D32(64), KGE_D4(96)
+               : "r"(a[0]), "r"(a[1]), "r"(a[2]), "r"(a[3]), "l"(bdesc), "r"(accumulate));
+}
+template <>
+__device__ __forceinline__ void wgmma_rs<208>(float (&d)[104], const uint32_t (&a)[4], uint64_t bdesc, uint32_t accumulate) {
+  asm volatile("{\n\t.reg .pred p;\n\tsetp.ne.b32 p, %109, 0;\n\t"
+               "wgmma.mma_async.sync.aligned.m64n208k8.f32.tf32.tf32 {%0,%1,%2,%3,%4,%5,%6,%7,%8,%9,%10,%11,%12,%13,%14,%15,%16,%17,%18,%19,%20,%21,%22,%23,%24,%25,%26,%27,%28,%29,%30,%31,%32,%33,%34,%35,%36,%37,%38,%39,%40,%41,%42,%43,%44,%45,%46,%47,%48,%49,%50,%51,%52,%53,%54,%55,%56,%57,%58,%59,%60,%61,%62,%63,%64,%65,%66,%67,%68,%69,%70,%71,%72,%73,%74,%75,%76,%77,%78,%79,%80,%81,%82,%83,%84,%85,%86,%87,%88,%89,%90,%91,%92,%93,%94,%95,%96,%97,%98,%99,%100,%101,%102,%103}, {%104,%105,%106,%107}, %108, p, 1, 1;\n\t}"
+               : KGE_D32(0), KGE_D32(32), KGE_D32(64), KGE_D4(96), KGE_D4(100)
+               : "r"(a[0]), "r"(a[1]), "r"(a[2]), "r"(a[3]), "l"(bdesc), "r"(accumulate));
+}
+template <>
+__device__ __forceinline__ void wgmma_rs<256>(float (&d)[128], const uint32_t (&a)[4], uint64_t bdesc, uint32_t accumulate) {
+  asm volatile("{\n\t.reg .pred p;\n\tsetp.ne.b32 p, %133, 0;\n\t"
+               "wgmma.mma_async.sync.aligned.m64n256k8.f32.tf32.tf32 {%0,%1,%2,%3,%4,%5,%6,%7,%8,%9,%10,%11,%12,%13,%14,%15,%16,%17,%18,%19,%20,%21,%22,%23,%24,%25,%26,%27,%28,%29,%30,%31,%32,%33,%34,%35,%36,%37,%38,%39,%40,%41,%42,%43,%44,%45,%46,%47,%48,%49,%50,%51,%52,%53,%54,%55,%56,%57,%58,%59,%60,%61,%62,%63,%64,%65,%66,%67,%68,%69,%70,%71,%72,%73,%74,%75,%76,%77,%78,%79,%80,%81,%82,%83,%84,%85,%86,%87,%88,%89,%90,%91,%92,%93,%94,%95,%96,%97,%98,%99,%100,%101,%102,%103,%104,%105,%106,%107,%108,%109,%110,%111,%112,%113,%114,%115,%116,%117,%118,%119,%120,%121,%122,%123,%124,%125,%126,%127}, {%128,%129,%130,%131}, %132, p, 1, 1;\n\t}"
+               : KGE_D32(0), KGE_D32(32), KGE_D32(64), KGE_D32(96)
                : "r"(a[0]), "r"(a[1]), "r"(a[2]), "r"(a[3]), "l"(bdesc), "r"(accumulate));
 }
 #undef KGE_D4
```

Result: faster. 33.19 million (median of 6 runs) (+7.5%).
